# Keytoyze/Mug-Diffusion

Hardware: NVIDIA H100
Metric: denoising-steps/sec (higher is better)
Workload: dtype f32

## Files before the change

### include/mugd.h

```cpp
#ifndef MUGD_H
#define MUGD_H

#include <stdint.h>

#ifdef __cplusplus
extern "C" {
#endif

#define MUGD_ABI_VERSION 13

typedef struct mugd_handle mugd_handle;
typedef struct mugd_plan mugd_plan;

enum mugd_status {
    MUGD_OK = 0,
    MUGD_ERR_INVALID = 1,
    MUGD_ERR_CUDA = 2,
    MUGD_ERR_NO_DEVICE = 3,
    MUGD_ERR_OOM = 4
};

enum mugd_op_kind {
    MUGD_OP_GEMM = 1,
    MUGD_OP_GROUPNORM = 2,
    MUGD_OP_LAYERNORM = 3,
    MUGD_OP_ATTENTION = 4,
    MUGD_OP_S4CONV = 5,
    MUGD_OP_DDIM_UPDATE = 6,
    MUGD_OP_TRANSPOSE = 7,
    MUGD_OP_COPY2D = 8,
    MUGD_OP_STEP_ADVANCE = 9,
    MUGD_OP_NOTES = 10,
    MUGD_OP_EMBED = 11,
    MUGD_OP_TF32_SPLIT = 12,
    MUGD_OP_POSTERIOR = 13
};

enum mugd_conv_mode {
    MUGD_CONV_NONE = 0,
    MUGD_CONV_SAME = 1,
    MUGD_CONV_DOWN = 2,
    MUGD_CONV_UP = 3,
    MUGD_CONV_TAPS = 4
};
enum mugd_act { MUGD_ACT_NONE = 0, MUGD_ACT_SILU = 1, MUGD_ACT_GELU = 2 };
enum mugd_gate { MUGD_GATE_NONE = 0, MUGD_GATE_GEGLU = 1 ,
                 MUGD_GATE_GLU = 2  };
enum mugd_gemm_impl { MUGD_GEMM_AUTO = 0, MUGD_GEMM_SIMT = 1 ,
                      MUGD_GEMM_TC = 2  };

typedef struct mugd_gemm {
    const float* A;  int64_t lda;
    const float* W;
    const float* W_hi;
    const float* W_lo;
    const float* bias;
    const float* rowvec;
    int64_t rowvec_b_stride;
    int64_t rowvec_step_stride;
    const int32_t* step;
    const float* residual; int64_t ldr;
    float* C;        int64_t ldc;
    int32_t M, N, K;
    int32_t taps, conv_mode, Lin, Lout;
    int32_t act, gate, impl;
    int32_t split_k;
    int32_t n_counters;
    int32_t tap_shift;
    int32_t tap_dilation;
    void* workspace; int64_t workspace_bytes;
    int32_t* counters;
    const float* A2; int64_t lda2;
    int32_t K2; int32_t reserved_;
    double* row_moments;
    const double* ln_stats; const float* ln_colsum; float ln_eps; int32_t reserved2_;
} mugd_gemm;

typedef struct mugd_groupnorm {
    const float* x; int64_t ldx; float* y; int64_t ldy;
    const float* gamma; const float* beta;
    int32_t B, L, C, G; float eps; int32_t silu;
} mugd_groupnorm;

typedef struct mugd_layernorm {
    const float* x; int64_t ldx; float* y; int64_t ldy;
    const float* gamma; const float* beta;
    int32_t rows, C; float eps;
} mugd_layernorm;

typedef struct mugd_attention {
    const float* q; int64_t ldq;
    const float* k; int64_t ldk;
    const float* v; int64_t ldv;
    float* o; int64_t ldo;
    const float* relpos;
    const float* cgain;
    int32_t B, H, D, Lq, Lk, pos_max; float scale;
} mugd_attention;

typedef struct mugd_s4conv {
    const float* u; int64_t ldu;
    const float* Kt;
    const float* D;
    float* y; int64_t ldy;
    int32_t B, L, H;
} mugd_s4conv;

typedef struct mugd_ddim_update {
    float* x;
    float* x_dup;
    const float* eps;
    const float* noise;
    float* pred_x0;
    const float* coef;
    const int32_t* step;
    int32_t S; int32_t n;
    int32_t cfg; float scale; float temperature;
} mugd_ddim_update;

typedef struct mugd_transpose {
    const float* in; float* out;
    int64_t ldi, ldo; int32_t B, C, L, to_nlc;
} mugd_transpose;

typedef struct mugd_copy2d {
    const float* src; int64_t lds; float* dst; int64_t ldd; int32_t rows, cols;
} mugd_copy2d;

typedef struct mugd_step_advance { int32_t* step; } mugd_step_advance;

typedef struct mugd_notes {
    const float* logits; int64_t ld;
    int32_t* count; int32_t* start_ms; int32_t* end_ms;
    double frame_ms;
    int32_t B, T, K;
} mugd_notes;

typedef struct mugd_embed {
    const float* table;
    const int32_t* ids;
    float* out;
    int32_t B, F, H, n_embed;
} mugd_embed;

typedef struct mugd_tf32_split { float* w_hi; float* lo; int64_t n; } mugd_tf32_split;

typedef struct mugd_posterior {
    const float* params;
    const float* noise;
    float *mean, *logvar, *std, *z;
    float scale;
    int32_t B, Z, L;
} mugd_posterior;

typedef struct mugd_op {
    int32_t kind;
    int32_t tag;
    union {
        mugd_gemm gemm; mugd_groupnorm gn; mugd_layernorm ln; mugd_attention attn; mugd_s4conv s4;
        mugd_ddim_update ddim; mugd_transpose tr; mugd_copy2d cp; mugd_step_advance adv; mugd_notes notes;
        mugd_embed embed; mugd_tf32_split split; mugd_posterior post;
    } u;
} mugd_op;

int  mugd_abi_version(void);
const char* mugd_last_error(void);
int  mugd_create(int device, mugd_handle** out);
void mugd_destroy(mugd_handle* h);
int  mugd_device_info(mugd_handle* h, int32_t* sm_count, int32_t* cc_major, int32_t* cc_minor);
int  mugd_set_gemm_impl(mugd_handle* h, int impl);
int  mugd_set_pdl(int enabled);

int  mugd_op_run(mugd_handle* h, const mugd_op* op, void* stream);

int  mugd_plan_create(mugd_handle* h, const mugd_op* ops, int32_t n_ops, mugd_plan** out);
int  mugd_plan_run(mugd_plan* p, void* stream);
int  mugd_plan_capture(mugd_plan* p, void* stream);
int  mugd_plan_replay(mugd_plan* p, int32_t times, void* stream);
int  mugd_plan_launch_count(mugd_plan* p);
void mugd_plan_destroy(mugd_plan* p);

int  mugd_sample(mugd_plan* eval_plan, const mugd_op* tail, int32_t n_tail, int32_t n_steps, void* stream);

typedef struct mugd_stage {
    float* x; float* x_dup;
    const float* x0;
    const float* mask;
    const float* q_noise;
    const float* q_coef;
    const float* noise;
    float* noise_rows;
    int32_t B, C, L, reserved_;
} mugd_stage;
int  mugd_sample_staged(mugd_plan* eval_plan, const mugd_stage* stage, const mugd_op* tail, int32_t n_tail, int32_t n_steps,
                        void* stream);

typedef struct mugd_plms {
    mugd_ddim_update update;
    const float* eps;
    float* e_prime;
    float* hist;
    float* x_stash;
    int32_t cfg; float scale;
} mugd_plms;
int  mugd_sample_plms(mugd_plan* eval_plan, const mugd_plms* p, int32_t first_step, int32_t n_steps, void* stream);
int  mugd_plms_combine(const mugd_plms* p, int32_t step, int32_t heun, void* stream);

#define MUGD_MAX_STEPS 1000
typedef struct mugd_ddpm {
    float* x; float* x_dup;
    const float* eps;
    float* pred_x0;
    const float* noise;
    const float* coef;
    int32_t* step;
    int32_t T, B, C, L;
    int32_t cfg; float scale;
    int32_t clip;
    int32_t reserved_;
} mugd_ddpm;
int  mugd_sample_ddpm(mugd_plan* eval_plan, const mugd_ddpm* d, int32_t first_step, int32_t n_steps, void* stream);
int  mugd_ddpm_update(const mugd_ddpm* d, void* stream);

typedef struct mugd_dpm {
    float* x; float* x_dup;
    const float* eps;
    float* pred_x0;
    float* ring;
    const float* coef;
    int32_t* step;
    int32_t n, S;
    int32_t cfg; float scale;
} mugd_dpm;
int  mugd_sample_dpm(mugd_plan* eval_plan, const mugd_dpm* d, int32_t first_step, int32_t n_steps, void* stream);
int  mugd_dpm_update(const mugd_dpm* d, void* stream);

typedef struct mugd_dpm_ex {
    mugd_dpm dpm;
    const mugd_stage* stage;
    const int32_t* start;
    const float* order_coef;
    int32_t B, reserved_;
} mugd_dpm_ex;
int  mugd_sample_dpm_ex(mugd_plan* eval_plan, const mugd_dpm_ex* e, int32_t first_step, int32_t n_steps, void* stream);
int  mugd_dpm_ex_update(const mugd_dpm_ex* e, void* stream);

typedef struct mugd_dpm_stop {
    mugd_dpm dpm;
    const int32_t* stop;
    int32_t B, reserved_;
} mugd_dpm_stop;
int  mugd_sample_dpm_stop(mugd_plan* eval_plan, const mugd_dpm_stop* e, int32_t first_step, int32_t n_steps, void* stream);
int  mugd_dpm_stop_update(const mugd_dpm_stop* e, void* stream);

typedef struct mugd_unipc {
    mugd_dpm dpm;
    float* xc;
    const float* corr;
} mugd_unipc;
int  mugd_sample_unipc(mugd_plan* eval_plan, const mugd_unipc* u, int32_t first_step, int32_t n_steps, void* stream);
int  mugd_unipc_update(const mugd_unipc* u, void* stream);

typedef struct mugd_unipc_ex {
    mugd_unipc unipc;
    const mugd_stage* stage;
    const int32_t* start;
    const float* order_coef;
    const float* order_corr;
    int32_t B, reserved_;
} mugd_unipc_ex;
int  mugd_sample_unipc_ex(mugd_plan* eval_plan, const mugd_unipc_ex* e, int32_t first_step, int32_t n_steps, void* stream);
int  mugd_unipc_ex_update(const mugd_unipc_ex* e, void* stream);

typedef struct mugd_unipc_stop {
    mugd_unipc unipc;
    const int32_t* stop;
    int32_t B, reserved_;
} mugd_unipc_stop;
int  mugd_sample_unipc_stop(mugd_plan* eval_plan, const mugd_unipc_stop* e, int32_t first_step, int32_t n_steps, void* stream);
int  mugd_unipc_stop_update(const mugd_unipc_stop* e, void* stream);

typedef struct mugd_q_encode {
    const float* x0; const float* noise;
    const int64_t* t;
    const float* sqrt_a; const float* sqrt_1ma;
    float* out;
    int32_t B, C, L, n;
} mugd_q_encode;
int  mugd_stochastic_encode(const mugd_q_encode* d, void* stream);

typedef struct mugd_join {
    float* x; float* x_dup;
    const float* x_latent;
    const int32_t* join;
    int32_t B, C, L, reserved_;
} mugd_join;
int  mugd_sample_join(mugd_plan* eval_plan, const mugd_join* join, const mugd_op* tail, int32_t n_tail, int32_t first_step,
                      int32_t n_steps, void* stream);

typedef struct mugd_region { const char* name; void* base; int64_t bytes; } mugd_region;
int  mugd_plan_save(mugd_plan* p, const mugd_region* regions, int32_t n_regions, const char* path);
int  mugd_plan_load(mugd_handle* h, const char* path, const mugd_region* regions, int32_t n_regions, mugd_plan** out);
int  mugd_plan_ops(mugd_plan* p, const mugd_op** ops, int32_t* n_ops);
int  mugd_plan_regions(const char* path, mugd_region* out, char (*names)[48], int32_t max_regions, int32_t* n_regions);

int  mugd_s4_kernel_gen(mugd_handle* h,
                        const float* log_dt,
                        const float* Bri,
                        const float* Cri,
                        const float* Pri,
                        const float* inv_w_real,
                        const float* w_imag,
                        const float* omega_ri,
                        int32_t H, int32_t N, int32_t L_internal, int32_t L_out,
                        float* Kt,
                        void* workspace, int64_t workspace_bytes,
                        void* stream);

int  mugd_melspec(mugd_handle* h,
                  const float* y, int64_t n, int64_t ldy, int32_t B,
                  const double* window, const double* twiddle, int32_t n_fft,
                  const int32_t* band_start, const int32_t* band_len, const float* weights, int32_t n_mels,
                  int32_t hop,
                  float* out, int64_t ldo, int32_t T_out,
                  void* stream);

int  mugd_grid_scan(mugd_handle* h, const float* times, const int32_t* chart_start, int32_t n_charts,
                    const double* cands, int32_t n_cands,
                    const int32_t* k0, const int32_t* head_len, const double* best_off, const double* best_score,
                    const float* first, const double* head_bpm, const double* head_off,
                    void* workspace, int32_t* out_i, double* out_d, void* stream);

int  mugd_chart_snap(mugd_handle* h, const int32_t* times, const int32_t* chart_start, int32_t n_charts,
                     const double* bpm, const double* offset, const int32_t* offset_is_f32, int64_t* out, void* stream);

int  mugd_remove_mini_jacks(mugd_handle* h, const int32_t* chart_start, int32_t n_charts, double jack_interval,
                            const double* start, const double* end, const uint8_t* is_long, int32_t* x, uint8_t* state,
                            void* workspace, void* stream);

int  mugd_gemm_tc_query(mugd_handle* h, const mugd_gemm* g, int32_t sm_count, int32_t* supported, int32_t* splits,
                        int64_t* workspace_bytes, int32_t* n_tiles);
int  mugd_gemm_tc_variant(const mugd_gemm* g, int32_t sm_count, int32_t* tile_n, int32_t* ctas_per_sm, int32_t* grid_ctas);

int  mugd_set_tc_single_pass_tf32(mugd_handle* h, int enabled);

int  mugd_set_attention_impl(mugd_handle* h, int impl);

int  mugd_set_s4conv_impl(mugd_handle* h, int impl);

int  mugd_debug_set_tc_cost(float kstep128_us, float kstep256_us, float split_us, float two_cta_fixed_us);

int  mugd_debug_set_tc_tile_n(int bn);

int  mugd_debug_set_attention_dump(float* buf);

int  mugd_debug_set_tc_timing(long long* device_buf);

int  mugd_fill_i32(int32_t* dst, int32_t value, void* stream);
int  mugd_abi_sizes(int32_t* out, int32_t n);

#ifdef __cplusplus
}
#endif
#endif
```

### mug_diffusion_b200/csrc/gemm_tc.cu

```cuda
#include "gemm_tc.cuh"

namespace mugd {

template <int BN, int EPI>
__global__ void __launch_bounds__(TC_THREADS, 1)
gemm_tc_kernel(const __grid_constant__ CUtensorMap tmA, const __grid_constant__ CUtensorMap tmA1,
               const __grid_constant__ CUtensorMap tmA2, const __grid_constant__ CUtensorMap tmB, const __grid_constant__ CUtensorMap tmWhi,
               const __grid_constant__ CUtensorMap tmWlo, const __grid_constant__ TcParams p) {
    extern __shared__ uint8_t smem_raw[];
    const uint32_t base = (smem_u32(smem_raw) + 1023u) & ~1023u;
    const TcBars<BN> B(base);
    TC_STAMP(p, 0, blockIdx.x == 0 && blockIdx.y == 0 && blockIdx.z == 0);
    if (threadIdx.x < 32) {
        B.init_parallel((int)threadIdx.x);
    } else if (threadIdx.x < 38) {
        const CUtensorMap* m = threadIdx.x == 32 ? &tmA : threadIdx.x == 33 ? &tmA1 : threadIdx.x == 34 ? &tmA2
                             : threadIdx.x == 35 ? &tmB : threadIdx.x == 36 ? &tmWhi : &tmWlo;
        asm volatile("prefetch.tensormap [%0];" ::"l"(reinterpret_cast<uint64_t>(m)) : "memory");
    }
    __syncthreads();
    TC_STAMP(p, 1, blockIdx.x == 0 && blockIdx.y == 0 && blockIdx.z == 0);
    gemm_tc_tile<BN, EPI>(&tmA, &tmA1, &tmA2, &tmB, &tmWhi, &tmWlo, p, blockIdx.x, blockIdx.y, blockIdx.z, base);
}

template <int BN, int EPI>
__global__ void __launch_bounds__(TC_THREADS)
gemm_tc_reduce_kernel(const __grid_constant__ TcParams p) {
    tc_reduce<BN, EPI>(p, blockIdx.x);
}

#ifdef MUGD_TC_TIMELINE
static long long* g_tc_dbg = nullptr;
#endif
static float g_tc_kstep128 = 0.55f;
static float g_tc_split = 3.0f;
static int g_tc_force_bn = 0;

static bool tc_shape_ok(const mugd_gemm& g) {
    if (!(g.conv_mode == MUGD_CONV_NONE || g.conv_mode == MUGD_CONV_SAME || g.conv_mode == MUGD_CONV_DOWN ||
          g.conv_mode == MUGD_CONV_TAPS)) return false;
    if (g.conv_mode == MUGD_CONV_DOWN && g.Lout < 2) return false;
    if (g.K2 % TC_BK != 0 || (g.K2 > 0 && g.conv_mode == MUGD_CONV_DOWN)) return false;
    return g.K % TC_BK == 0 && g.N >= 16 && g.N % 4 == 0;
}

bool gemm_tc_supported(const mugd_gemm& g) {
    if (!tc_shape_ok(g)) return false;
    if (!g.W_hi || !g.W_lo) return false;
    if (g.lda % 4 != 0 || !aligned16(g.A) || !aligned16(g.W_hi) || !aligned16(g.W_lo)) return false;
    if (g.K2 > 0 && (!g.A2 || g.lda2 % 4 != 0 || !aligned16(g.A2))) return false;
    return true;
}

static int tc_validate_fusions(const mugd_gemm& g) {
    if (g.row_moments)
        MUGD_REQUIRE(g.act == MUGD_ACT_NONE && g.gate == MUGD_GATE_NONE && !g.ln_stats && (reinterpret_cast<uintptr_t>(g.row_moments) & 15u) == 0,
                     "gemm: row_moments needs act == gate == NONE, no folded LayerNorm and a 16-byte aligned buffer");
    if (g.ln_stats) {
        MUGD_REQUIRE(g.ln_colsum && aligned16(g.ln_colsum) && (reinterpret_cast<uintptr_t>(g.ln_stats) & 15u) == 0 && g.taps == 1 && g.K2 == 0 &&
                         g.act == MUGD_ACT_NONE && (g.gate == MUGD_GATE_NONE || g.gate == MUGD_GATE_GEGLU) && !g.rowvec,
                     "gemm: folded LayerNorm needs a single-source Linear with act NONE and gate NONE/GEGLU");
    }
    return MUGD_OK;
}

TcGeometry tc_geometry(const mugd_gemm& g, int sm_count, int forced_split) {
    TcGeometry t = {};
    TcParams::Hot& h = t.hot;
    t.BN = (g.N >= 128) ? 128 : 64;
    if (g.conv_mode == MUGD_CONV_NONE) { h.Lrows = g.M; h.Bs = 1; }
    else { h.Lrows = g.Lout; h.Bs = g.M / g.Lout; }
    if (h.Lrows >= TC_BM) {
        h.box_l = TC_BM; h.box_b = 1;
        h.tiles_per_sample = (h.Lrows + TC_BM - 1) / TC_BM;
        t.gy = h.tiles_per_sample * h.Bs;
    } else {
        h.box_l = h.Lrows;
        h.box_b = TC_BM / h.Lrows;
        if (h.box_b > h.Bs) h.box_b = h.Bs;
        h.tiles_per_sample = 1;
        t.gy = (h.Bs + h.box_b - 1) / h.box_b;
    }
    h.kblocks = g.K / TC_BK;
    h.it_main = g.taps * h.kblocks;
    h.total_it = h.it_main + g.K2 / TC_BK;
    int splits = 1;
    float best = 1e30f;
    static const int cands[2] = {64, 128};
    for (int cand = 0; cand < 2; ++cand) {
        const int bn = cands[cand];
        if (bn > 64 && g.N < bn) continue;
        if (bn == 64 && g.N >= 128 && g_tc_force_bn != 64) continue;
        if (g_tc_force_bn && bn != g_tc_force_bn && !(g_tc_force_bn > g.N && bn == 64)) continue;
        const int gx = (g.N + bn - 1) / bn;
        const int tiles = gx * t.gy;
        const float kstep = bn == 128 ? g_tc_kstep128 : 0.4f;
        const int sp_max = forced_split > 0 ? forced_split : (tiles < sm_count ? 16 : 1);
        for (int sp = forced_split > 0 ? forced_split : 1; sp <= sp_max && sp <= h.total_it; ++sp) {
            const int per = (h.total_it + sp - 1) / sp;
            if (forced_split <= 0 && sp > 1 && per < 2) break;
            if (forced_split <= 0 && sp > 1 && tiles * sp > 2 * sm_count) break;
            const int waves = (tiles * sp + sm_count - 1) / sm_count;
            const float est = waves * (1.0f + kstep * per) + (sp > 1 ? g_tc_split : 0.0f);
            if (est < best - 0.25f) { best = est; splits = sp; t.BN = bn; }
        }
    }
    h.gx = (g.N + t.BN - 1) / t.BN;
    if (splits > h.total_it) splits = h.total_it;
    if (splits < 1) splits = 1;
    h.splits = splits;
    h.it_base = h.total_it / splits;
    h.it_rem = h.total_it % splits;
    h.conv_mode = g.conv_mode;
    h.tap_shift = g.tap_shift;
    h.tap_dilation = g.tap_dilation;
    t.ws_floats = splits > 1 ? (int64_t)h.gx * t.gy * splits * TC_BM * t.BN : 0;
    return t;
}

int tc_plan(const DeviceInfo& dev, const mugd_gemm& g, const mugd_gemm* next, TcPlanned* out) {
    MUGD_REQUIRE(gemm_tc_supported(g), "gemm_tc: unsupported shape/operands");
    int rc = tc_validate_fusions(g);
    if (rc != MUGD_OK) return rc;
    const TcGeometry t = tc_geometry(g, dev.sm_count, g.split_k);
    const TcParams::Hot& h = t.hot;
    if (h.splits > 1) {
        MUGD_REQUIRE(g.workspace, "gemm_tc: split-K needs a workspace");
        MUGD_REQUIRE(g.workspace_bytes >= t.ws_floats * 4, "gemm_tc: workspace too small (%lld < %lld)", (long long)g.workspace_bytes,
                     (long long)t.ws_floats * 4);
    }
    const cuuint32_t a_box[3] = {(cuuint32_t)TC_BK, (cuuint32_t)h.box_l, (cuuint32_t)h.box_b};
    for (int tap = 0; tap < 3; ++tap) {
        if (tap > 0 && g.conv_mode != MUGD_CONV_DOWN) { out->maps[tap] = out->maps[0]; continue; }
        const bool down = g.conv_mode == MUGD_CONV_DOWN;
        const cuuint64_t rows = down ? (cuuint64_t)(h.Lrows - (tap == 2 ? 1 : 0)) : (cuuint64_t)h.Lrows;
        const cuuint64_t sample_rows = down ? (cuuint64_t)g.Lin : (cuuint64_t)h.Lrows;
        const cuuint64_t dims[3] = {(cuuint64_t)g.K, rows, (cuuint64_t)h.Bs};
        const cuuint64_t strides[2] = {(cuuint64_t)g.lda * 4 * (down ? 2 : 1), sample_rows * (cuuint64_t)g.lda * 4};
        rc = encode_f32_tma(&out->maps[tap], g.A + (down ? (int64_t)tap * g.lda : 0), 3, dims, strides, a_box, CU_TENSOR_MAP_L2_PROMOTION_L2_128B,
                            "gemm_tc A");
        if (rc != MUGD_OK) return rc;
    }
    if (g.K2 > 0) {
        const cuuint64_t dims[3] = {(cuuint64_t)g.K2, (cuuint64_t)h.Lrows, (cuuint64_t)h.Bs};
        const cuuint64_t strides[2] = {(cuuint64_t)g.lda2 * 4, (cuuint64_t)h.Lrows * (cuuint64_t)g.lda2 * 4};
        rc = encode_f32_tma(&out->maps[3], g.A2, 3, dims, strides, a_box, CU_TENSOR_MAP_L2_PROMOTION_L2_128B, "gemm_tc A2");
        if (rc != MUGD_OK) return rc;
    } else {
        out->maps[3] = out->maps[0];
    }
    const cuuint64_t ktot = (cuuint64_t)g.taps * g.K + g.K2;
    const cuuint64_t w_dims[2] = {ktot, (cuuint64_t)g.N};
    const cuuint64_t w_strides[1] = {ktot * 4};
    const cuuint32_t w_box[2] = {(cuuint32_t)TC_BK, (cuuint32_t)t.BN};
    for (int w = 0; w < 2; ++w) {
        rc = encode_f32_tma(&out->maps[4 + w], w == 0 ? g.W_hi : g.W_lo, 2, w_dims, w_strides, w_box, CU_TENSOR_MAP_L2_PROMOTION_L2_256B,
                            "gemm_tc W");
        if (rc != MUGD_OK) return rc;
    }
    TcParams& p = out->p;
    memset(&p, 0, sizeof(p));
    p.hot = h;
    p.hot.single_pass = dev.tc_single_pass ? 1 : 0;
    p.g = g;
    p.ws = (float*)g.workspace;
    p.gy = t.gy;
    p.ln_invK = 1.0 / (double)g.K;
    if (next) {
        p.pf_hi = next->W_hi;
        p.pf_lo = p.hot.single_pass ? nullptr : next->W_lo;
        p.pf_bytes = (int64_t)next->N * ((int64_t)next->taps * next->K + next->K2) * 4;
    }
#ifdef MUGD_TC_TIMELINE
    p.dbg = g_tc_dbg;
#endif
    out->BN = t.BN;
    return MUGD_OK;
}

template <int BN, int EPI>
static int tc_launch(const TcPlanned& pl, cudaStream_t st) {
    const TcParams& p = pl.p;
    const TcParams::Hot& h = p.hot;
    if (h.splits > 1) {
        MUGD_CHECK_CUDA(launch_k(gemm_tc_kernel<BN, TC_E_NONE>, dim3(h.gx, p.gy, h.splits), dim3(TC_THREADS), TcSmem<BN>::TOTAL, st, pl.maps[0],
                                 pl.maps[1], pl.maps[2], pl.maps[3], pl.maps[4], pl.maps[5], p));
        MUGD_CHECK_CUDA(launch_k(gemm_tc_reduce_kernel<BN, EPI>, dim3((unsigned)(h.gx * p.gy * (TC_BM / TC_RED_ROWS<BN>))), dim3(TC_THREADS), 0,
                                 st, p));
        return MUGD_OK;
    }
    MUGD_CHECK_CUDA(launch_k(gemm_tc_kernel<BN, EPI>, dim3(h.gx, p.gy, 1), dim3(TC_THREADS), TcSmem<BN>::TOTAL, st, pl.maps[0], pl.maps[1],
                             pl.maps[2], pl.maps[3], pl.maps[4], pl.maps[5], p));
    return MUGD_OK;
}

template <int BN, int... EPI>
static cudaError_t allow_smem_bn(int bytes, std::integer_sequence<int, EPI...>) {
    return allow_dynamic_smem(bytes, gemm_tc_kernel<BN, EPI>...);
}
cudaError_t gemm_tc_allow_smem(int bytes) {
    const cudaError_t e = allow_smem_bn<64>(bytes, std::make_integer_sequence<int, TC_E_COUNT>{});
    return e != cudaSuccess ? e : allow_smem_bn<128>(bytes, std::make_integer_sequence<int, TC_E_COUNT>{});
}

template <int BN>
static int tc_launch_bn(const TcPlanned& pl, cudaStream_t st) {
    switch (tc_epi_of(pl.p.g)) {
        case TC_E_GEGLU: return tc_launch<BN, TC_E_GEGLU>(pl, st);
        case TC_E_GLU: return tc_launch<BN, TC_E_GLU>(pl, st);
        case TC_E_SILU: return tc_launch<BN, TC_E_SILU>(pl, st);
        case TC_E_GELU: return tc_launch<BN, TC_E_GELU>(pl, st);
        case TC_E_SINK: return tc_launch<BN, TC_E_SINK>(pl, st);
        case TC_E_LN: return tc_launch<BN, TC_E_LN>(pl, st);
        case TC_E_LN_GEGLU: return tc_launch<BN, TC_E_LN_GEGLU>(pl, st);
        default: return tc_launch<BN, TC_E_NONE>(pl, st);
    }
}

int launch_gemm_tc(const DeviceInfo& dev, const mugd_gemm& g, const mugd_gemm* next, cudaStream_t st, int* launches) {
    TcPlanned pl;
    int rc = tc_plan(dev, g, next, &pl);
    if (rc != MUGD_OK) return rc;
    if (pl.BN == 128) rc = tc_launch_bn<128>(pl, st);
    else rc = tc_launch_bn<64>(pl, st);
    if (rc != MUGD_OK) return rc;
    if (launches) *launches += pl.p.hot.splits > 1 ? 2 : 1;
    return MUGD_OK;
}

}

extern "C" int mugd_debug_set_tc_cost(float kstep128_us, float kstep256_us, float split_us, float two_cta_fixed_us) {
    (void)kstep256_us;
    (void)two_cta_fixed_us;
    if (kstep128_us > 0.f) mugd::g_tc_kstep128 = kstep128_us;
    if (split_us > 0.f) mugd::g_tc_split = split_us;
    return MUGD_OK;
}

extern "C" int mugd_debug_set_tc_tile_n(int bn) {
    mugd::g_tc_force_bn = (bn == 64 || bn == 128) ? bn : 0;
    return MUGD_OK;
}

extern "C" int mugd_debug_set_tc_timing(long long* device_buf) {
#ifdef MUGD_TC_TIMELINE
    mugd::g_tc_dbg = device_buf;
    return MUGD_OK;
#else
    (void)device_buf;
    mugd::set_error("mugd_debug_set_tc_timing: this build has no timeline hooks (rebuild with -DMUGD_TC_TIMELINE, tools/build_variant.py)");
    return MUGD_ERR_INVALID;
#endif
}

extern "C" int mugd_gemm_tc_variant(const mugd_gemm* g, int32_t sm_count, int32_t* tile_n, int32_t* ctas_per_sm, int32_t* grid_ctas) {
    using namespace mugd;
    MUGD_REQUIRE(g, "gemm_tc_variant: null");
    if (!tc_shape_ok(*g)) {
        if (tile_n) *tile_n = 0;
        if (ctas_per_sm) *ctas_per_sm = 0;
        if (grid_ctas) *grid_ctas = 0;
        return MUGD_OK;
    }
    const int sms = sm_count > 0 ? sm_count : 132;
    const TcGeometry t = tc_geometry(*g, sms, g->split_k);
    if (tile_n) *tile_n = t.BN;
    if (ctas_per_sm) *ctas_per_sm = 1;
    if (grid_ctas) *grid_ctas = t.hot.gx * t.gy * t.hot.splits;
    return MUGD_OK;
}

extern "C" int mugd_gemm_tc_query(mugd_handle*, const mugd_gemm* g, int32_t sm_count, int32_t* supported, int32_t* splits,
                                  int64_t* workspace_bytes, int32_t* n_tiles) {
    using namespace mugd;
    MUGD_REQUIRE(g, "gemm_tc_query: null");
    const bool ok = tc_shape_ok(*g);
    if (supported) *supported = ok ? 1 : 0;
    if (!ok) {
        if (splits) *splits = 0;
        if (workspace_bytes) *workspace_bytes = 0;
        if (n_tiles) *n_tiles = 0;
        return MUGD_OK;
    }
    const TcGeometry t = tc_geometry(*g, sm_count > 0 ? sm_count : 132, g->split_k);
    if (splits) *splits = t.hot.splits;
    if (workspace_bytes) *workspace_bytes = t.ws_floats * 4;
    if (n_tiles) *n_tiles = t.hot.gx * t.gy;
    return MUGD_OK;
}
```

### mug_diffusion_b200/csrc/gemm_tc.cuh

```cuda
#pragma once
#include <cuda.h>
#include <stddef.h>

#include <type_traits>

#include "common.cuh"
#include "wgmma.cuh"

namespace mugd {

constexpr int TC_BM = 128;
constexpr int TC_BK = 32;
constexpr int TC_THREADS = 256;
constexpr uint32_t TC_A_BYTES = TC_BM * TC_BK * 4;

struct TcParams {
    struct Hot {
        int32_t Lrows, Bs;
        int32_t box_l, box_b;
        int32_t tiles_per_sample;
        int32_t it_base, it_rem;
        int32_t it_main;
        int32_t kblocks;
        int32_t total_it;
        int32_t splits;
        int32_t single_pass;
        int32_t conv_mode, tap_shift, tap_dilation;
        int32_t gx;
    } hot;
    mugd_gemm g;
    float* ws;
    int32_t gy;
    double ln_invK;
    const float* pf_hi;
    const float* pf_lo;
    int64_t pf_bytes;
#ifdef MUGD_TC_TIMELINE
    long long* dbg;
#endif
};
static_assert(sizeof(TcParams::Hot) == 64 && offsetof(TcParams, hot) == 0, "the hot fields are the first 64 bytes of the parameters");

#ifdef __CUDACC__
__device__ __forceinline__ long long gtimer() {
    long long t;
    asm volatile("mov.u64 %0, %%globaltimer;" : "=l"(t) :: "memory");
    return t;
}
#ifdef MUGD_TC_TIMELINE
#define TC_STAMP(p, k, cta0) do { if ((p).dbg && (cta0) && threadIdx.x == 0) (p).dbg[k] = gtimer(); } while (0)
#else
#define TC_STAMP(p, k, cta0) do { } while (0)
#endif
template <int BN>
struct TcSmem {
    static_assert(BN == 64 || BN == 128, "tile widths of the wgmma kernel");
    static constexpr uint32_t B_BYTES = BN * TC_BK * 4;
    static constexpr uint32_t STAGE_BYTES = TC_A_BYTES + 2 * B_BYTES;
    static constexpr int STAGES = BN == 128 ? 4 : 6;
    static constexpr uint32_t TILE_BYTES = STAGES * STAGE_BYTES;
    static constexpr uint32_t BAR_BYTES = 256;
    static constexpr uint32_t TOTAL = TILE_BYTES + 1024  + BAR_BYTES;
    static_assert(TOTAL <= 227u * 1024u, "shared memory budget");
    static_assert(128u * (BN + 4) * 4u + 1024u <= TILE_BYTES, "the staged accumulator tile + row statistics must fit the pipeline buffers");
};

template <int SEG>
__device__ __forceinline__ void tc_row_sink(double* buf, int m, float4 v) {
    float s = (v.x + v.y) + (v.z + v.w);
    float ss = (v.x * v.x + v.y * v.y) + (v.z * v.z + v.w * v.w);
#pragma unroll
    for (int o = SEG / 2; o > 0; o >>= 1) {
        s += __shfl_xor_sync(0xffffffffu, s, o);
        ss += __shfl_xor_sync(0xffffffffu, ss, o);
    }
    if ((threadIdx.x & (SEG - 1)) == 0 && m >= 0) {
        atomicAdd(buf + (int64_t)m * 2, (double)s);
        atomicAdd(buf + (int64_t)m * 2 + 1, (double)ss);
    }
}
__device__ __forceinline__ float2 tc_ln_from_moments(double s, double ss, double invK, float eps) {
    const double mean = s * invK;
    double var = ss * invK - mean * mean;
    const float v = fmaxf((float)var, 0.f) + eps;
    float r = rsqrtf(v);
    r = r * (1.5f - 0.5f * v * r * r);
    return make_float2((float)mean, r);
}

constexpr int TC_EPI_PLAIN = 0, TC_EPI_SINK = 1 , TC_EPI_LN = 2 ;

template <int ACT, int GATE, bool LNF>
__device__ __forceinline__ float4 tc_finish4(const mugd_gemm& g, float* dst, float4 acc, float4 bia, float4 rvv, float4 res, float4 cs, float2 ln,
                                             int m, int no) {
    float x[4];
    if constexpr (LNF) {
        x[0] = (acc.x - ln.x * cs.x) * ln.y + bia.x + rvv.x; x[1] = (acc.y - ln.x * cs.y) * ln.y + bia.y + rvv.y;
        x[2] = (acc.z - ln.x * cs.z) * ln.y + bia.z + rvv.z; x[3] = (acc.w - ln.x * cs.w) * ln.y + bia.w + rvv.w;
    } else {
        x[0] = acc.x + bia.x + rvv.x; x[1] = acc.y + bia.y + rvv.y; x[2] = acc.z + bia.z + rvv.z; x[3] = acc.w + bia.w + rvv.w;
    }
    if constexpr (ACT == MUGD_ACT_SILU) {
#pragma unroll
        for (int j = 0; j < 4; ++j) x[j] = silu_f(x[j]);
    } else if constexpr (ACT == MUGD_ACT_GELU) {
#pragma unroll
        for (int j = 0; j < 4; ++j) x[j] = gelu_f(x[j]);
    }
    if constexpr (GATE == MUGD_GATE_NONE) {
        const float4 o = make_float4(x[0] + res.x, x[1] + res.y, x[2] + res.z, x[3] + res.w);
        st_f4(dst, o);
        return o;
    } else {
        float o0, o1;
        if constexpr (GATE == MUGD_GATE_GEGLU) { o0 = x[0] * gelu_f(x[1]); o1 = x[2] * gelu_f(x[3]); }
        else { o0 = x[0] * sigmoid_f(x[1]); o1 = x[2] * sigmoid_f(x[3]); }
        if (g.residual) {
            const float2 rr = *reinterpret_cast<const float2*>(g.residual + (int64_t)m * g.ldr + no);
            o0 += rr.x; o1 += rr.y;
        }
        *reinterpret_cast<float2*>(dst) = make_float2(o0, o1);
        return make_float4(o0, o1, 0.f, 0.f);
    }
}

template <int BN, int ACT, int GATE, int MODE>
__device__ __forceinline__ void tc_store_tile(const mugd_gemm& g, uint32_t stage, int m_base, int n0, int rows_valid, const float* rowvec,
                                              uint32_t rowstat, float4 bia, float4 cs) {
    constexpr int SP = BN + 4;
    constexpr int C4 = BN / 4;
    constexpr int NU = TC_BM * C4 / TC_THREADS;
    constexpr int U = NU < 16 ? NU : 16;
    constexpr int SEG = C4 < 32 ? C4 : 32;
    static_assert(TC_THREADS % C4 == 0, "a thread keeps its column quad for the whole tile");
    const int c4 = (int)threadIdx.x % C4;
    const int nn = n0 + c4 * 4;
    const bool col_ok = nn < g.N;
    const bool has_res = GATE == MUGD_GATE_NONE && g.residual != nullptr;
    constexpr int RPP = TC_THREADS / C4;
    const int row0 = (int)threadIdx.x / C4;
    const int n_rows = min(rows_valid, g.M - m_base);
    const int no = (GATE == MUGD_GATE_NONE) ? nn : (nn >> 1);
    float* cp = g.C + (int64_t)(m_base + row0) * g.ldc + no;
    const float* rp = has_res ? g.residual + (int64_t)(m_base + row0) * g.ldr + nn : nullptr;
    const int64_t c_step = (int64_t)RPP * g.ldc, r_step = (int64_t)RPP * g.ldr;
    int smp = 0, smp_end = 0;
    if (rowvec) { smp = (m_base + row0) / g.Lout; smp_end = (smp + 1) * g.Lout; }
    auto pass = [&](auto full_tag) {
        constexpr bool FULL = decltype(full_tag)::value;
#pragma unroll 1
        for (int i0 = 0; i0 < NU; i0 += U) {
            float4 res[U], rvv[U];
#pragma unroll
            for (int u = 0; u < U; ++u) {
                const int row = row0 + (i0 + u) * RPP;
                res[u] = rvv[u] = make_float4(0.f, 0.f, 0.f, 0.f);
                if (FULL || (row < n_rows && col_ok)) {
                    if (has_res) res[u] = ld_f4(rp + (int64_t)(i0 + u) * r_step);
                    if (rowvec) {
                        const int m = m_base + row;
                        while (m >= smp_end) { ++smp; smp_end += g.Lout; }
                        rvv[u] = ld_f4(rowvec + (int64_t)smp * g.rowvec_b_stride + nn);
                    }
                }
            }
#pragma unroll
            for (int u = 0; u < U; ++u) {
                const int row = row0 + (i0 + u) * RPP;
                const int m = m_base + row;
                const bool ok = FULL || (row < n_rows && col_ok);
                const float4 acc = lds_f4(stage + (uint32_t)(row * SP + c4 * 4) * 4u);
                float2 ln = make_float2(0.f, 1.f);
                if constexpr (MODE == TC_EPI_LN) ln = lds_f2(rowstat + (uint32_t)row * 8u);
                float4 o = make_float4(0.f, 0.f, 0.f, 0.f);
                if (ok) o = tc_finish4<ACT, GATE, MODE == TC_EPI_LN>(g, cp + (int64_t)(i0 + u) * c_step, acc, bia, rvv[u], res[u], cs, ln, m, no);
                if constexpr (MODE == TC_EPI_SINK) tc_row_sink<SEG>(g.row_moments, ok ? m : -1, o);
            }
        }
    };
    if (n_rows >= TC_BM && n0 + BN <= g.N) pass(std::true_type{});
    else pass(std::false_type{});
}

enum TcEpi { TC_E_NONE = 0, TC_E_GEGLU, TC_E_GLU, TC_E_SILU, TC_E_GELU, TC_E_SINK, TC_E_LN, TC_E_LN_GEGLU, TC_E_COUNT };
template <int EPI> struct TcEpiTraits;
template <> struct TcEpiTraits<TC_E_NONE>     { static constexpr int ACT = MUGD_ACT_NONE, GATE = MUGD_GATE_NONE,  MODE = TC_EPI_PLAIN; };
template <> struct TcEpiTraits<TC_E_GEGLU>    { static constexpr int ACT = MUGD_ACT_NONE, GATE = MUGD_GATE_GEGLU, MODE = TC_EPI_PLAIN; };
template <> struct TcEpiTraits<TC_E_GLU>      { static constexpr int ACT = MUGD_ACT_NONE, GATE = MUGD_GATE_GLU,   MODE = TC_EPI_PLAIN; };
template <> struct TcEpiTraits<TC_E_SILU>     { static constexpr int ACT = MUGD_ACT_SILU, GATE = MUGD_GATE_NONE,  MODE = TC_EPI_PLAIN; };
template <> struct TcEpiTraits<TC_E_GELU>     { static constexpr int ACT = MUGD_ACT_GELU, GATE = MUGD_GATE_NONE,  MODE = TC_EPI_PLAIN; };
template <> struct TcEpiTraits<TC_E_SINK>     { static constexpr int ACT = MUGD_ACT_NONE, GATE = MUGD_GATE_NONE,  MODE = TC_EPI_SINK; };
template <> struct TcEpiTraits<TC_E_LN>       { static constexpr int ACT = MUGD_ACT_NONE, GATE = MUGD_GATE_NONE,  MODE = TC_EPI_LN; };
template <> struct TcEpiTraits<TC_E_LN_GEGLU> { static constexpr int ACT = MUGD_ACT_NONE, GATE = MUGD_GATE_GEGLU, MODE = TC_EPI_LN; };

inline int tc_epi_of(const mugd_gemm& g) {
    if (g.ln_stats) return g.gate == MUGD_GATE_GEGLU ? TC_E_LN_GEGLU : TC_E_LN;
    if (g.row_moments) return TC_E_SINK;
    if (g.gate == MUGD_GATE_GEGLU) return TC_E_GEGLU;
    if (g.gate == MUGD_GATE_GLU) return TC_E_GLU;
    if (g.act == MUGD_ACT_SILU) return TC_E_SILU;
    if (g.act == MUGD_ACT_GELU) return TC_E_GELU;
    return TC_E_NONE;
}

__device__ __forceinline__ void tc_tile_rows(const TcParams& p, int by, int& b_base, int& l_base, int& rows_valid) {
    const TcParams::Hot& h = p.hot;
    if (h.Lrows >= TC_BM) {
        b_base = by / h.tiles_per_sample;
        l_base = (by % h.tiles_per_sample) * TC_BM;
        rows_valid = min(TC_BM, h.Lrows - l_base);
    } else {
        b_base = by * h.box_b;
        l_base = 0;
        rows_valid = min(h.box_b, h.Bs - b_base) * h.Lrows;
    }
}

template <int BN>
struct TcBars {
    using S = TcSmem<BN>;
    static constexpr int COUNT = 2 * S::STAGES;
    static_assert(8 * COUNT <= (int)S::BAR_BYTES, "barrier block");
    uint32_t bars;
    __device__ __forceinline__ explicit TcBars(uint32_t base) : bars(base + S::TILE_BYTES) {}
    __device__ __forceinline__ uint32_t full(int s) const { return bars + 8u * s; }
    __device__ __forceinline__ uint32_t empty(int s) const { return bars + 8u * (S::STAGES + s); }
    __device__ __forceinline__ void init_parallel(int t) const {
        if (t >= COUNT) return;
        mbar_init(bars + 8u * t, t < S::STAGES ? 1u : (uint32_t)(TC_THREADS / 32));
        mbar_init_fence();
    }
};

struct TcAFrag {
    uint32_t hi[4][4], lo[4][4];
};
__device__ __forceinline__ void tc_load_split(uint32_t a_tile, int r0, int t, TcAFrag& f) {
#pragma unroll
    for (int kk = 0; kk < 4; ++kk) {
#pragma unroll
        for (int e = 0; e < 4; ++e) {
            const int r = r0 + (e & 1) * 8;
            const int chunk = 2 * kk + (e >> 1);
            const float x = lds_f1(a_tile + (uint32_t)r * 128u + (uint32_t)((chunk ^ (r & 7)) << 4) + (uint32_t)t * 4u);
            const float h = to_tf32(x);
            f.hi[kk][e] = __float_as_uint(h);
            f.lo[kk][e] = __float_as_uint(to_tf32(x - h));
        }
    }
}

template <int BN, int EPI>
__device__ __forceinline__ void gemm_tc_tile(const CUtensorMap* tmA, const CUtensorMap* tmA1, const CUtensorMap* tmA2, const CUtensorMap* tmB,
                                             const CUtensorMap* tmWhi, const CUtensorMap* tmWlo, const TcParams& p, int bx, int by, int bz,
                                             uint32_t base) {
    using S = TcSmem<BN>;
    constexpr int STAGES = S::STAGES;
    constexpr int NACC = BN / 2;
    const TcBars<BN> B(base);
    auto a_raw = [&](int s) { return base + s * S::STAGE_BYTES; };
    auto b_hi = [&](int s) { return base + s * S::STAGE_BYTES + TC_A_BYTES; };
    auto b_lo = [&](int s) { return b_hi(s) + S::B_BYTES; };

    const mugd_gemm& g = p.g;
    const TcParams::Hot& h = p.hot;
    const int warp = threadIdx.x >> 5, lane = threadIdx.x & 31;
    const int n0 = bx * BN;
    int b_base, l_base, rows_valid;
    tc_tile_rows(p, by, b_base, l_base, rows_valid);
    const int m_base = b_base * h.Lrows + l_base;
    const int it_begin = bz * h.it_base + min(bz, h.it_rem);
    const int nit = h.it_base + (bz < h.it_rem ? 1 : 0);
    const uint32_t a_tx = (uint32_t)(h.box_l * h.box_b) * TC_BK * 4;
    const uint32_t w_tx = (h.single_pass ? 1u : 2u) * S::B_BYTES;

    auto issue_w = [&](int i) {
        const int s = i % STAGES, it = it_begin + i;
        mbar_expect_tx(B.full(s), a_tx + w_tx);
        tma_load_2d(b_hi(s), tmWhi, B.full(s), it * TC_BK, n0);
        if (!h.single_pass) tma_load_2d(b_lo(s), tmWlo, B.full(s), it * TC_BK, n0);
    };
    auto issue_a = [&](int i) {
        const int s = i % STAGES, it = it_begin + i;
        if (it < h.it_main) {
            const int t = it / h.kblocks;
            const int kb = it - t * h.kblocks;
            const CUtensorMap* ma = tmA;
            int lshift = 0;
            if (h.conv_mode == MUGD_CONV_SAME) lshift = t - 1;
            else if (h.conv_mode == MUGD_CONV_TAPS) lshift = (t + h.tap_shift) * (h.tap_dilation > 1 ? h.tap_dilation : 1);
            else if (h.conv_mode == MUGD_CONV_DOWN) ma = (t == 0) ? tmA : (t == 1 ? tmA1 : tmA2);
            tma_load_3d(a_raw(s), ma, B.full(s), kb * TC_BK, l_base + lshift, b_base);
        } else {
            tma_load_3d(a_raw(s), tmB, B.full(s), (it - h.it_main) * TC_BK, l_base, b_base);
        }
    };
    if (warp == 0) {
        if (elect_one()) {
            const int pro = nit < STAGES ? nit : STAGES;
            for (int i = 0; i < pro; ++i) issue_w(i);
            pdl_wait();
            for (int i = 0; i < pro; ++i) issue_a(i);
            if (p.pf_bytes > 0) {
                const int64_t ncta = (int64_t)h.gx * p.gy * h.splits;
                const int64_t per = (p.pf_bytes / ncta + 15) & ~(int64_t)15;
                const int64_t off = (((int64_t)bz * p.gy + by) * h.gx + bx) * per;
                const int64_t n = min(per, p.pf_bytes - off);
                if (n > 0) {
                    prefetch_l2(reinterpret_cast<const char*>(p.pf_hi) + off, (uint32_t)n);
                    if (p.pf_lo) prefetch_l2(reinterpret_cast<const char*>(p.pf_lo) + off, (uint32_t)n);
                }
            }
        }
        __syncwarp();
    }

    int epi_step = 0;
    float4 epi_bias = make_float4(0.f, 0.f, 0.f, 0.f), epi_cs = epi_bias;
    double ln_s = 0.0, ln_ss = 0.0;
    {
        pdl_wait();
        if (h.splits == 1) {
            const int nn = n0 + ((int)threadIdx.x % (BN / 4)) * 4;
            if (g.step) epi_step = *g.step;
            if (g.bias && nn < g.N) epi_bias = ld_f4(g.bias + nn);
            if constexpr (TcEpiTraits<EPI>::MODE == TC_EPI_LN) {
                if (nn < g.N) epi_cs = ld_f4(g.ln_colsum + nn);
            }
        }
        if constexpr (TcEpiTraits<EPI>::MODE == TC_EPI_LN) {
            const int rr = (int)threadIdx.x;
            if (rr < TC_BM && rr < rows_valid && m_base + rr < g.M) {
                const double2 mo = *reinterpret_cast<const double2*>(g.ln_stats + (int64_t)m_base * 2 + rr * 2);
                ln_s = mo.x; ln_ss = mo.y;
            }
        }
    }

    const int wg = warp >> 2, g8 = lane >> 2, t4 = lane & 3;
    const int r0 = wg * 64 + (warp & 3) * 16 + g8;
    float acc[NACC];
#pragma unroll
    for (int j = 0; j < NACC; ++j) acc[j] = 0.f;
    TcAFrag f0, f1;
    if (nit > 0) {
        mbar_wait(B.full(0), 0u);
        tc_load_split(a_raw(0), r0, t4, f0);
    }
    auto main_loop = [&](auto single_tag) {
        constexpr bool SINGLE = decltype(single_tag)::value;
        auto kstep = [&](int i, const TcAFrag& cur, TcAFrag& nxt) {
            const int s = i % STAGES;
            const uint64_t dbh = wgmma_desc(b_hi(s)), dbl = wgmma_desc(b_lo(s));
            wgmma_fence();
#pragma unroll
            for (int kk = 0; kk < TC_BK / 8; ++kk) {
                const uint64_t ko = (uint64_t)(kk * 2);
                if constexpr (SINGLE) {
                    Wgmma<BN>::mma(acc, cur.hi[kk], dbh + ko);
                } else {
                    Wgmma<BN>::mma(acc, cur.lo[kk], dbh + ko);
                    Wgmma<BN>::mma(acc, cur.hi[kk], dbl + ko);
                    Wgmma<BN>::mma(acc, cur.hi[kk], dbh + ko);
                }
            }
            wgmma_commit();
            wgmma_wait<1>();
            if (i > 0) {
                const int j = i - 1, sj = j % STAGES;
                __syncwarp();
                if (lane == 0) mbar_arrive(B.empty(sj));
                if (warp == 0 && j + STAGES < nit) {
                    mbar_wait(B.empty(sj), (uint32_t)(j / STAGES) & 1u);
                    if (elect_one()) { issue_w(j + STAGES); issue_a(j + STAGES); }
                    __syncwarp();
                }
            }
            if (i + 1 < nit) {
                mbar_wait(B.full((i + 1) % STAGES), (uint32_t)((i + 1) / STAGES) & 1u);
                tc_load_split(a_raw((i + 1) % STAGES), r0, t4, nxt);
            }
        };
        for (int i = 0; i < nit; i += 2) {
            kstep(i, f0, f1);
            if (i + 1 < nit) kstep(i + 1, f1, f0);
        }
    };
    if (h.single_pass) main_loop(std::true_type{});
    else main_loop(std::false_type{});
    wgmma_wait<0>();
    TC_STAMP(p, 2, bx == 0 && by == 0 && bz == 0);
    float2 lnrow = make_float2(0.f, 1.f);
    if constexpr (TcEpiTraits<EPI>::MODE == TC_EPI_LN) lnrow = tc_ln_from_moments(ln_s, ln_ss, p.ln_invK, g.ln_eps);
    __syncthreads();
    constexpr int SP = BN + 4;
#pragma unroll
    for (int j = 0; j < BN / 8; ++j) {
        const int c = j * 8 + 2 * t4;
        sts_f2(base + (uint32_t)(r0 * SP + c) * 4u, acc[4 * j], acc[4 * j + 1]);
        sts_f2(base + (uint32_t)((r0 + 8) * SP + c) * 4u, acc[4 * j + 2], acc[4 * j + 3]);
    }
    if constexpr (TcEpiTraits<EPI>::MODE == TC_EPI_LN) {
        if (threadIdx.x < TC_BM) sts_f2(base + S::TILE_BYTES - 1024u + (uint32_t)threadIdx.x * 8u, lnrow.x, lnrow.y);
    }
    __syncthreads();
    TC_STAMP(p, 3, bx == 0 && by == 0 && bz == 0);
    {
        const float* rowvec = g.rowvec ? g.rowvec + (int64_t)epi_step * g.rowvec_step_stride : nullptr;
        if (h.splits > 1) {
            const int tile_lin = by * h.gx + bx;
            float* wsp = p.ws + ((int64_t)tile_lin * h.splits + bz) * (TC_BM * BN);
            constexpr int C4 = BN / 4;
            constexpr int U = 8;
#pragma unroll 1
            for (int i0 = 0; i0 < TC_BM * C4; i0 += TC_THREADS * U) {
                float4 a4[U];
#pragma unroll
                for (int u = 0; u < U; ++u) {
                    const int idx = i0 + u * TC_THREADS + (int)threadIdx.x;
                    const int row = idx / C4, c4 = idx - row * C4;
                    a4[u] = lds_f4(base + (uint32_t)(row * SP + c4 * 4) * 4u);
                }
#pragma unroll
                for (int u = 0; u < U; ++u) st_f4(wsp + (i0 + u * TC_THREADS + (int)threadIdx.x) * 4, a4[u]);
            }
        } else {
            using E = TcEpiTraits<EPI>;
            tc_store_tile<BN, E::ACT, E::GATE, E::MODE>(g, base, m_base, n0, rows_valid, rowvec, base + S::TILE_BYTES - 1024u, epi_bias, epi_cs);
        }
    }
    TC_STAMP(p, 4, bx == 0 && by == 0 && bz == 0);
}

template <int BN> constexpr int TC_RED_ROWS = TC_THREADS / (BN / 4);

template <int BN, int EPI>
__device__ __forceinline__ void tc_reduce(const TcParams& p, int blk) {
    constexpr int ACT = TcEpiTraits<EPI>::ACT, GATE = TcEpiTraits<EPI>::GATE, MODE = TcEpiTraits<EPI>::MODE;
    constexpr int C4 = BN / 4;
    constexpr int BPT = TC_BM / TC_RED_ROWS<BN>;
    constexpr int SEG = C4 < 32 ? C4 : 32;
    constexpr int ZU = 8;
    const mugd_gemm& g = p.g;
    const TcParams::Hot& h = p.hot;
    const int tile_lin = blk / BPT;
    const int bx = tile_lin % h.gx, by = tile_lin / h.gx;
    int b_base, l_base, rows_valid;
    tc_tile_rows(p, by, b_base, l_base, rows_valid);
    const int m_base = b_base * h.Lrows + l_base;
    const int c4 = (int)threadIdx.x % C4;
    const int r = (blk % BPT) * TC_RED_ROWS<BN> + (int)threadIdx.x / C4;
    const int n = bx * BN + c4 * 4;
    const int m = m_base + r;
    const bool ok = r < rows_valid && m < g.M && n < g.N;
    float4 bia = make_float4(0.f, 0.f, 0.f, 0.f), rvv = bia, res = bia, cs = bia;
    if (ok && g.bias) bia = ld_f4(g.bias + n);
    if constexpr (MODE == TC_EPI_LN) {
        if (ok) cs = ld_f4(g.ln_colsum + n);
    }
    pdl_wait();
    int step = 0;
    if (g.step) step = *g.step;
    if (GATE == MUGD_GATE_NONE && g.residual && ok) res = ld_f4(g.residual + (int64_t)m * g.ldr + n);
    double2 mo = make_double2(0.0, 1.0);
    if constexpr (MODE == TC_EPI_LN) {
        if (ok) mo = *reinterpret_cast<const double2*>(g.ln_stats + (int64_t)m * 2);
    }
    const float* src = p.ws + ((long long)tile_lin * h.splits) * (TC_BM * BN) + (long long)r * BN + c4 * 4;
    float4 acc = make_float4(0.f, 0.f, 0.f, 0.f);
    for (int z0 = 0; z0 < h.splits; z0 += ZU) {
        float4 t4[ZU];
#pragma unroll
        for (int u = 0; u < ZU; ++u) {
            t4[u] = make_float4(0.f, 0.f, 0.f, 0.f);
            if (ok && z0 + u < h.splits) t4[u] = __ldcg(reinterpret_cast<const float4*>(src + (long long)(z0 + u) * (TC_BM * BN)));
        }
        if (z0 == 0 && g.rowvec && ok)
            rvv = ld_f4(g.rowvec + (int64_t)step * g.rowvec_step_stride + (int64_t)(m / g.Lout) * g.rowvec_b_stride + n);
#pragma unroll
        for (int u = 0; u < ZU; ++u) { acc.x += t4[u].x; acc.y += t4[u].y; acc.z += t4[u].z; acc.w += t4[u].w; }
    }
    float4 o = make_float4(0.f, 0.f, 0.f, 0.f);
    if (ok) {
        float2 ln = make_float2(0.f, 1.f);
        if constexpr (MODE == TC_EPI_LN) ln = tc_ln_from_moments(mo.x, mo.y, p.ln_invK, g.ln_eps);
        const int no = (GATE == MUGD_GATE_NONE) ? n : (n >> 1);
        o = tc_finish4<ACT, GATE, MODE == TC_EPI_LN>(g, g.C + (int64_t)m * g.ldc + no, acc, bia, rvv, res, cs, ln, m, no);
    }
    if constexpr (MODE == TC_EPI_SINK) tc_row_sink<SEG>(g.row_moments, ok ? m : -1, o);
}

#endif

struct TcGeometry {
    TcParams::Hot hot;
    int BN, gy;
    int64_t ws_floats;
};
struct alignas(64) TcPlanned {
    CUtensorMap maps[6];
    TcParams p;
    int BN;
};
TcGeometry tc_geometry(const mugd_gemm& g, int sm_count, int forced_split);
int tc_plan(const DeviceInfo& dev, const mugd_gemm& g, const mugd_gemm* next, TcPlanned* out);

}
```

### mug_diffusion_b200/lib.py

```python
from __future__ import annotations

import ctypes as C
import os
from typing import Optional

HERE = os.path.dirname(os.path.abspath(__file__))
LIB_PATH = os.environ.get("MUGD_LIB") or os.path.join(HERE, "libmugd.so")

(OP_GEMM, OP_GROUPNORM, OP_LAYERNORM, OP_ATTENTION, OP_S4CONV, OP_DDIM_UPDATE, OP_TRANSPOSE, OP_COPY2D, OP_STEP_ADVANCE, OP_NOTES, OP_EMBED,
 OP_TF32_SPLIT, OP_POSTERIOR) = range(1, 14)
CONV_NONE, CONV_SAME, CONV_DOWN, CONV_UP, CONV_TAPS = range(5)
ACT_NONE, ACT_SILU, ACT_GELU = range(3)
GATE_NONE, GATE_GEGLU, GATE_GLU = range(3)
GEMM_AUTO, GEMM_SIMT, GEMM_TC = range(3)
ABI_VERSION = 13

_f = C.c_void_p


class Gemm(C.Structure):
    _fields_ = [("A", _f), ("lda", C.c_int64), ("W", _f), ("W_hi", _f), ("W_lo", _f), ("bias", _f), ("rowvec", _f),
                ("rowvec_b_stride", C.c_int64), ("rowvec_step_stride", C.c_int64), ("step", _f),
                ("residual", _f), ("ldr", C.c_int64), ("C", _f), ("ldc", C.c_int64),
                ("M", C.c_int32), ("N", C.c_int32), ("K", C.c_int32),
                ("taps", C.c_int32), ("conv_mode", C.c_int32), ("Lin", C.c_int32), ("Lout", C.c_int32),
                ("act", C.c_int32), ("gate", C.c_int32), ("impl", C.c_int32),
                ("split_k", C.c_int32), ("n_counters", C.c_int32), ("tap_shift", C.c_int32), ("tap_dilation", C.c_int32),
                ("workspace", _f), ("workspace_bytes", C.c_int64), ("counters", _f),
                ("A2", _f), ("lda2", C.c_int64), ("K2", C.c_int32), ("reserved_", C.c_int32),
                ("row_moments", _f),
                ("ln_stats", _f), ("ln_colsum", _f), ("ln_eps", C.c_float), ("reserved2_", C.c_int32)]


class GroupNorm(C.Structure):
    _fields_ = [("x", _f), ("ldx", C.c_int64), ("y", _f), ("ldy", C.c_int64), ("gamma", _f), ("beta", _f),
                ("B", C.c_int32), ("L", C.c_int32), ("C", C.c_int32), ("G", C.c_int32),
                ("eps", C.c_float), ("silu", C.c_int32)]


class LayerNorm(C.Structure):
    _fields_ = [("x", _f), ("ldx", C.c_int64), ("y", _f), ("ldy", C.c_int64), ("gamma", _f), ("beta", _f),
                ("rows", C.c_int32), ("C", C.c_int32), ("eps", C.c_float)]


class Attention(C.Structure):
    _fields_ = [("q", _f), ("ldq", C.c_int64), ("k", _f), ("ldk", C.c_int64), ("v", _f), ("ldv", C.c_int64),
                ("o", _f), ("ldo", C.c_int64), ("relpos", _f), ("cgain", _f),
                ("B", C.c_int32), ("H", C.c_int32), ("D", C.c_int32), ("Lq", C.c_int32), ("Lk", C.c_int32),
                ("pos_max", C.c_int32), ("scale", C.c_float)]


class S4Conv(C.Structure):
    _fields_ = [("u", _f), ("ldu", C.c_int64), ("Kt", _f), ("D", _f), ("y", _f), ("ldy", C.c_int64),
                ("B", C.c_int32), ("L", C.c_int32), ("H", C.c_int32)]


class DdimUpdate(C.Structure):
    _fields_ = [("x", _f), ("x_dup", _f), ("eps", _f), ("noise", _f), ("pred_x0", _f), ("coef", _f), ("step", _f),
                ("S", C.c_int32), ("n", C.c_int32), ("cfg", C.c_int32), ("scale", C.c_float),
                ("temperature", C.c_float)]


class Transpose(C.Structure):
    _fields_ = [("inp", _f), ("out", _f), ("ldi", C.c_int64), ("ldo", C.c_int64),
                ("B", C.c_int32), ("C", C.c_int32), ("L", C.c_int32), ("to_nlc", C.c_int32)]


class Copy2D(C.Structure):
    _fields_ = [("src", _f), ("lds", C.c_int64), ("dst", _f), ("ldd", C.c_int64),
                ("rows", C.c_int32), ("cols", C.c_int32)]


class StepAdvance(C.Structure):
    _fields_ = [("step", _f)]


class Notes(C.Structure):
    _fields_ = [("logits", _f), ("ld", C.c_int64), ("count", _f), ("start_ms", _f), ("end_ms", _f), ("frame_ms", C.c_double),
                ("B", C.c_int32), ("T", C.c_int32), ("K", C.c_int32)]


class Embed(C.Structure):
    _fields_ = [("table", _f), ("ids", _f), ("out", _f), ("B", C.c_int32), ("F", C.c_int32), ("H", C.c_int32), ("n_embed", C.c_int32)]


class Tf32Split(C.Structure):
    _fields_ = [("w_hi", _f), ("lo", _f), ("n", C.c_int64)]


class Posterior(C.Structure):
    _fields_ = [("params", _f), ("noise", _f), ("mean", _f), ("logvar", _f), ("std", _f), ("z", _f), ("scale", C.c_float),
                ("B", C.c_int32), ("Z", C.c_int32), ("L", C.c_int32)]


class Stage(C.Structure):
    _fields_ = [("x", _f), ("x_dup", _f), ("x0", _f), ("mask", _f), ("q_noise", _f), ("q_coef", _f), ("noise", _f), ("noise_rows", _f),
                ("B", C.c_int32), ("C", C.c_int32), ("L", C.c_int32), ("reserved_", C.c_int32)]


class Plms(C.Structure):
    _fields_ = [("update", DdimUpdate), ("eps", _f), ("e_prime", _f), ("hist", _f), ("x_stash", _f), ("cfg", C.c_int32),
                ("scale", C.c_float)]


class Ddpm(C.Structure):
    _fields_ = [("x", _f), ("x_dup", _f), ("eps", _f), ("pred_x0", _f), ("noise", _f), ("coef", _f), ("step", _f),
                ("T", C.c_int32), ("B", C.c_int32), ("C", C.c_int32), ("L", C.c_int32), ("cfg", C.c_int32), ("scale", C.c_float),
                ("clip", C.c_int32), ("reserved_", C.c_int32)]


class Dpm(C.Structure):
    _fields_ = [("x", _f), ("x_dup", _f), ("eps", _f), ("pred_x0", _f), ("ring", _f), ("coef", _f), ("step", _f),
                ("n", C.c_int32), ("S", C.c_int32), ("cfg", C.c_int32), ("scale", C.c_float)]


class DpmEx(C.Structure):
    _fields_ = [("dpm", Dpm), ("stage", _f), ("start", _f), ("order_coef", _f), ("B", C.c_int32), ("reserved_", C.c_int32)]


class DpmStop(C.Structure):
    _fields_ = [("dpm", Dpm), ("stop", _f), ("B", C.c_int32), ("reserved_", C.c_int32)]


class Unipc(C.Structure):
    _fields_ = [("dpm", Dpm), ("xc", _f), ("corr", _f)]


class UnipcEx(C.Structure):
    _fields_ = [("unipc", Unipc), ("stage", _f), ("start", _f), ("order_coef", _f), ("order_corr", _f), ("B", C.c_int32),
                ("reserved_", C.c_int32)]


class UnipcStop(C.Structure):
    _fields_ = [("unipc", Unipc), ("stop", _f), ("B", C.c_int32), ("reserved_", C.c_int32)]


class QEncode(C.Structure):
    _fields_ = [("x0", _f), ("noise", _f), ("t", _f), ("sqrt_a", _f), ("sqrt_1ma", _f), ("out", _f),
                ("B", C.c_int32), ("C", C.c_int32), ("L", C.c_int32), ("n", C.c_int32)]


class Join(C.Structure):
    _fields_ = [("x", _f), ("x_dup", _f), ("x_latent", _f), ("join", _f),
                ("B", C.c_int32), ("C", C.c_int32), ("L", C.c_int32), ("reserved_", C.c_int32)]


class _OpU(C.Union):
    _fields_ = [("gemm", Gemm), ("gn", GroupNorm), ("ln", LayerNorm), ("attn", Attention), ("s4", S4Conv),
                ("ddim", DdimUpdate), ("tr", Transpose), ("cp", Copy2D), ("adv", StepAdvance), ("notes", Notes), ("embed", Embed),
                ("split", Tf32Split), ("post", Posterior)]


class Op(C.Structure):
    _fields_ = [("kind", C.c_int32), ("tag", C.c_int32), ("u", _OpU)]


_KIND_FIELD = {OP_GEMM: "gemm", OP_GROUPNORM: "gn", OP_LAYERNORM: "ln", OP_ATTENTION: "attn", OP_S4CONV: "s4",
               OP_DDIM_UPDATE: "ddim", OP_TRANSPOSE: "tr", OP_COPY2D: "cp", OP_STEP_ADVANCE: "adv", OP_NOTES: "notes", OP_EMBED: "embed", OP_TF32_SPLIT: "split",
               OP_POSTERIOR: "post"}


def make_op(kind: int, desc, tag: int = 0) -> Op:
    op = Op()
    op.kind = kind
    op.tag = tag
    setattr(op.u, _KIND_FIELD[kind], desc)
    return op


class Region(C.Structure):
    _fields_ = [("name", C.c_char_p), ("base", _f), ("bytes", C.c_int64)]


class MugdError(RuntimeError):
    pass


_lib: Optional[C.CDLL] = None


def load() -> C.CDLL:
    global _lib
    if _lib is not None:
        return _lib
    if not os.path.exists(LIB_PATH):
        raise MugdError(f"{LIB_PATH} not found: build it with `python -m mug_diffusion_b200.build` "
                        "(there is no CPU/PyTorch fallback for the sampler path)")
    lib = C.CDLL(LIB_PATH)
    lib.mugd_last_error.restype = C.c_char_p
    lib.mugd_abi_version.restype = C.c_int
    lib.mugd_create.argtypes = [C.c_int, C.POINTER(C.c_void_p)]
    lib.mugd_destroy.argtypes = [C.c_void_p]
    lib.mugd_destroy.restype = None
    lib.mugd_device_info.argtypes = [C.c_void_p, C.POINTER(C.c_int32), C.POINTER(C.c_int32), C.POINTER(C.c_int32)]
    lib.mugd_set_gemm_impl.argtypes = [C.c_void_p, C.c_int]
    lib.mugd_op_run.argtypes = [C.c_void_p, C.POINTER(Op), C.c_void_p]
    lib.mugd_plan_create.argtypes = [C.c_void_p, C.POINTER(Op), C.c_int32, C.POINTER(C.c_void_p)]
    lib.mugd_plan_run.argtypes = [C.c_void_p, C.c_void_p]
    lib.mugd_plan_capture.argtypes = [C.c_void_p, C.c_void_p]
    lib.mugd_plan_replay.argtypes = [C.c_void_p, C.c_int32, C.c_void_p]
    lib.mugd_plan_launch_count.argtypes = [C.c_void_p]
    lib.mugd_plan_destroy.argtypes = [C.c_void_p]
    lib.mugd_plan_destroy.restype = None
    lib.mugd_s4_kernel_gen.argtypes = [C.c_void_p] + [C.c_void_p] * 7 + [C.c_int32] * 4 + [C.c_void_p, C.c_void_p, C.c_int64, C.c_void_p]
    lib.mugd_melspec.argtypes = [C.c_void_p, C.c_void_p, C.c_int64, C.c_int64, C.c_int32, C.c_void_p, C.c_void_p, C.c_int32,
                                 C.POINTER(C.c_int32), C.POINTER(C.c_int32), C.c_void_p, C.c_int32, C.c_int32,
                                 C.c_void_p, C.c_int64, C.c_int32, C.c_void_p]
    lib.mugd_grid_scan.argtypes = [C.c_void_p, C.c_void_p, C.c_void_p, C.c_int32, C.c_void_p, C.c_int32] + [C.c_void_p] * 11
    lib.mugd_chart_snap.argtypes = [C.c_void_p, C.c_void_p, C.c_void_p, C.c_int32] + [C.c_void_p] * 5
    lib.mugd_remove_mini_jacks.argtypes = [C.c_void_p, C.c_void_p, C.c_int32, C.c_double] + [C.c_void_p] * 7
    lib.mugd_gemm_tc_variant.argtypes =[C.POINTER(Gemm), C.c_int32, C.POINTER(C.c_int32), C.POINTER(C.c_int32), C.POINTER(C.c_int32)]
    lib.mugd_gemm_tc_query.argtypes = [C.c_void_p, C.POINTER(Gemm), C.c_int32, C.POINTER(C.c_int32), C.POINTER(C.c_int32),
                                       C.POINTER(C.c_int64), C.POINTER(C.c_int32)]
    lib.mugd_set_pdl.argtypes = [C.c_int]
    lib.mugd_debug_set_tc_timing.argtypes = [C.c_void_p]
    lib.mugd_fill_i32.argtypes = [C.c_void_p, C.c_int32, C.c_void_p]
    lib.mugd_abi_sizes.argtypes = [C.POINTER(C.c_int32), C.c_int32]
    if lib.mugd_abi_version() != ABI_VERSION:
        raise MugdError(f"libmugd ABI {lib.mugd_abi_version()} != binding {ABI_VERSION}: rebuild the library")
    sizes = (C.c_int32 * 13)()
    lib.mugd_abi_sizes(sizes, 13)
    mine = [C.sizeof(t) for t in (Op, Gemm, GroupNorm, LayerNorm, Attention, S4Conv, DdimUpdate, Transpose, Copy2D, Notes, Embed, Tf32Split,
                                  Posterior)]
    if list(sizes) != mine:
        raise MugdError(f"struct layout mismatch: C {list(sizes)} vs ctypes {mine}")
    lib.mugd_sample.argtypes = [C.c_void_p, C.POINTER(Op), C.c_int32, C.c_int32, C.c_void_p]
    lib.mugd_sample_staged.argtypes = [C.c_void_p, C.POINTER(Stage), C.POINTER(Op), C.c_int32, C.c_int32, C.c_void_p]
    lib.mugd_sample_plms.argtypes = [C.c_void_p, C.POINTER(Plms), C.c_int32, C.c_int32, C.c_void_p]
    lib.mugd_plms_combine.argtypes = [C.POINTER(Plms), C.c_int32, C.c_int32, C.c_void_p]
    lib.mugd_sample_ddpm.argtypes = [C.c_void_p, C.POINTER(Ddpm), C.c_int32, C.c_int32, C.c_void_p]
    lib.mugd_ddpm_update.argtypes = [C.POINTER(Ddpm), C.c_void_p]
    lib.mugd_sample_dpm.argtypes = [C.c_void_p, C.POINTER(Dpm), C.c_int32, C.c_int32, C.c_void_p]
    lib.mugd_dpm_update.argtypes = [C.POINTER(Dpm), C.c_void_p]
    lib.mugd_sample_dpm_ex.argtypes = [C.c_void_p, C.POINTER(DpmEx), C.c_int32, C.c_int32, C.c_void_p]
    lib.mugd_dpm_ex_update.argtypes = [C.POINTER(DpmEx), C.c_void_p]
    lib.mugd_sample_dpm_stop.argtypes = [C.c_void_p, C.POINTER(DpmStop), C.c_int32, C.c_int32, C.c_void_p]
    lib.mugd_dpm_stop_update.argtypes = [C.POINTER(DpmStop), C.c_void_p]
    lib.mugd_sample_unipc.argtypes = [C.c_void_p, C.POINTER(Unipc), C.c_int32, C.c_int32, C.c_void_p]
    lib.mugd_unipc_update.argtypes = [C.POINTER(Unipc), C.c_void_p]
    lib.mugd_sample_unipc_ex.argtypes = [C.c_void_p, C.POINTER(UnipcEx), C.c_int32, C.c_int32, C.c_void_p]
    lib.mugd_unipc_ex_update.argtypes = [C.POINTER(UnipcEx), C.c_void_p]
    lib.mugd_sample_unipc_stop.argtypes = [C.c_void_p, C.POINTER(UnipcStop), C.c_int32, C.c_int32, C.c_void_p]
    lib.mugd_unipc_stop_update.argtypes = [C.POINTER(UnipcStop), C.c_void_p]
    lib.mugd_stochastic_encode.argtypes = [C.POINTER(QEncode), C.c_void_p]
    lib.mugd_sample_join.argtypes = [C.c_void_p, C.POINTER(Join), C.POINTER(Op), C.c_int32, C.c_int32, C.c_int32, C.c_void_p]
    lib.mugd_plan_save.argtypes = [C.c_void_p, C.POINTER(Region), C.c_int32, C.c_char_p]
    lib.mugd_plan_load.argtypes = [C.c_void_p, C.c_char_p, C.POINTER(Region), C.c_int32, C.POINTER(C.c_void_p)]
    lib.mugd_set_tc_single_pass_tf32.argtypes = [C.c_void_p, C.c_int]
    lib.mugd_set_attention_impl.argtypes = [C.c_void_p, C.c_int]
    lib.mugd_set_s4conv_impl.argtypes = [C.c_void_p, C.c_int]
    lib.mugd_debug_set_tc_tile_n.argtypes = [C.c_int]
    lib.mugd_debug_set_tc_cost.argtypes = [C.c_float, C.c_float, C.c_float, C.c_float]
    if os.environ.get("MUGD_TC_COST"):
        lib.mugd_debug_set_tc_cost(*([float(v) for v in os.environ["MUGD_TC_COST"].split(",")] + [0.0] * 4)[:4])
    if os.environ.get("MUGD_TC_TILE"):
        lib.mugd_debug_set_tc_tile_n(int(os.environ["MUGD_TC_TILE"]))
    if os.environ.get("MUGD_TC_BN"):
        lib.mugd_debug_set_tc_tile_n(int(os.environ["MUGD_TC_BN"]))
    if os.environ.get("MUGD_PDL") in ("0", "1"):
        lib.mugd_set_pdl(int(os.environ["MUGD_PDL"]))
    _lib = lib
    return lib


def check(rc: int, what: str = ""):
    if rc != 0:
        msg = load().mugd_last_error().decode(errors="replace")
        if rc == 4:
            import torch
            raise torch.cuda.OutOfMemoryError(f"{what}: {msg}")
        raise MugdError(f"{what} failed (status {rc}): {msg}")


EXPORTED_SYMBOLS = [
    "mugd_abi_version", "mugd_last_error", "mugd_create", "mugd_destroy", "mugd_device_info", "mugd_set_gemm_impl",
    "mugd_op_run", "mugd_plan_create", "mugd_plan_run", "mugd_plan_capture", "mugd_plan_replay",
    "mugd_plan_launch_count", "mugd_plan_destroy", "mugd_s4_kernel_gen", "mugd_fill_i32", "mugd_abi_sizes", "mugd_gemm_tc_query",
    "mugd_set_pdl", "mugd_set_tc_single_pass_tf32", "mugd_set_attention_impl", "mugd_set_s4conv_impl", "mugd_debug_set_tc_tile_n", "mugd_debug_set_tc_cost", "mugd_gemm_tc_variant",
    "mugd_debug_set_attention_dump", "mugd_debug_set_tc_timing", "mugd_sample", "mugd_plan_save", "mugd_plan_load", "mugd_plan_regions", "mugd_plan_ops",
    "mugd_melspec", "mugd_grid_scan", "mugd_chart_snap", "mugd_remove_mini_jacks",
    "mugd_sample_staged", "mugd_sample_plms", "mugd_plms_combine",
    "mugd_sample_ddpm", "mugd_ddpm_update", "mugd_stochastic_encode", "mugd_sample_join",
    "mugd_sample_dpm", "mugd_dpm_update", "mugd_sample_dpm_ex", "mugd_dpm_ex_update",
    "mugd_sample_dpm_stop", "mugd_dpm_stop_update",
    "mugd_sample_unipc", "mugd_unipc_update", "mugd_sample_unipc_ex", "mugd_unipc_ex_update",
    "mugd_sample_unipc_stop", "mugd_unipc_stop_update",
]
```

Measured before the change: 244.8.

## Add 256-row wgmma tile variant chosen by an L2-aware cost model

Adds a BM=256, BN=128 tile shape to the TF32 wgmma GEMM. Each warp holds two 64-row accumulator blocks so every weight tile loaded from shared memory is reused across twice as many rows. The geometry planner now compares 128- and 256-row candidates with a cost model that weighs tensor throughput against L2 bandwidth. The larger tile cuts the pipeline to 3 stages, raises register pressure, and is not split along K unless forced, which can reduce parallelism on small GEMMs.

```diff
diff --git a/include/mugd.h b/include/mugd.h
--- a/include/mugd.h
+++ b/include/mugd.h
@@ -352,6 +352,8 @@
 
 int  mugd_debug_set_tc_tile_n(int bn);
 
+int  mugd_debug_set_tc_tile_m(int bm);
+
 int  mugd_debug_set_attention_dump(float* buf);
 
 int  mugd_debug_set_tc_timing(long long* device_buf);
diff --git a/mug_diffusion_b200/csrc/gemm_tc.cu b/mug_diffusion_b200/csrc/gemm_tc.cu
--- a/mug_diffusion_b200/csrc/gemm_tc.cu
+++ b/mug_diffusion_b200/csrc/gemm_tc.cu
@@ -2,14 +2,14 @@
 
 namespace mugd {
 
-template <int BN, int EPI>
+template <int BM, int BN, int EPI>
 __global__ void __launch_bounds__(TC_THREADS, 1)
 gemm_tc_kernel(const __grid_constant__ CUtensorMap tmA, const __grid_constant__ CUtensorMap tmA1,
                const __grid_constant__ CUtensorMap tmA2, const __grid_constant__ CUtensorMap tmB, const __grid_constant__ CUtensorMap tmWhi,
                const __grid_constant__ CUtensorMap tmWlo, const __grid_constant__ TcParams p) {
     extern __shared__ uint8_t smem_raw[];
     const uint32_t base = (smem_u32(smem_raw) + 1023u) & ~1023u;
-    const TcBars<BN> B(base);
+    const TcBars<BM, BN> B(base);
     TC_STAMP(p, 0, blockIdx.x == 0 && blockIdx.y == 0 && blockIdx.z == 0);
     if (threadIdx.x < 32) {
         B.init_parallel((int)threadIdx.x);
@@ -20,13 +20,13 @@
     }
     __syncthreads();
     TC_STAMP(p, 1, blockIdx.x == 0 && blockIdx.y == 0 && blockIdx.z == 0);
-    gemm_tc_tile<BN, EPI>(&tmA, &tmA1, &tmA2, &tmB, &tmWhi, &tmWlo, p, blockIdx.x, blockIdx.y, blockIdx.z, base);
-}
-
-template <int BN, int EPI>
+    gemm_tc_tile<BM, BN, EPI>(&tmA, &tmA1, &tmA2, &tmB, &tmWhi, &tmWlo, p, blockIdx.x, blockIdx.y, blockIdx.z, base);
+}
+
+template <int BM, int BN, int EPI>
 __global__ void __launch_bounds__(TC_THREADS)
 gemm_tc_reduce_kernel(const __grid_constant__ TcParams p) {
-    tc_reduce<BN, EPI>(p, blockIdx.x);
+    tc_reduce<BM, BN, EPI>(p, blockIdx.x);
 }
 
 #ifdef MUGD_TC_TIMELINE
@@ -34,7 +34,10 @@
 #endif
 static float g_tc_kstep128 = 0.55f;
 static float g_tc_split = 3.0f;
+static float g_tc_tensor128_us = 0.78f;
+static float g_tc_l2_gbps = 5600.f;
 static int g_tc_force_bn = 0;
+static int g_tc_force_bm = 0;
 
 static bool tc_shape_ok(const mugd_gemm& g) {
     if (!(g.conv_mode == MUGD_CONV_NONE || g.conv_mode == MUGD_CONV_SAME || g.conv_mode == MUGD_CONV_DOWN ||
@@ -64,47 +67,64 @@
     return MUGD_OK;
 }
 
+static float tc_kstep_us(float tensor, float kbytes, int streams) {
+    const float l2 = kbytes * 1024.f * (float)streams / (g_tc_l2_gbps * 1e3f);
+    return tensor > l2 ? tensor : l2;
+}
+
 TcGeometry tc_geometry(const mugd_gemm& g, int sm_count, int forced_split) {
     TcGeometry t = {};
     TcParams::Hot& h = t.hot;
+    t.BM = 128;
     t.BN = (g.N >= 128) ? 128 : 64;
     if (g.conv_mode == MUGD_CONV_NONE) { h.Lrows = g.M; h.Bs = 1; }
     else { h.Lrows = g.Lout; h.Bs = g.M / g.Lout; }
-    if (h.Lrows >= TC_BM) {
-        h.box_l = TC_BM; h.box_b = 1;
-        h.tiles_per_sample = (h.Lrows + TC_BM - 1) / TC_BM;
-        t.gy = h.tiles_per_sample * h.Bs;
-    } else {
-        h.box_l = h.Lrows;
-        h.box_b = TC_BM / h.Lrows;
-        if (h.box_b > h.Bs) h.box_b = h.Bs;
-        h.tiles_per_sample = 1;
-        t.gy = (h.Bs + h.box_b - 1) / h.box_b;
-    }
+    auto row_tiles = [&](int bm) {
+        if (h.Lrows >= bm) return h.Bs * ((h.Lrows + bm - 1) / bm);
+        const int bb = bm / h.Lrows < h.Bs ? bm / h.Lrows : h.Bs;
+        return (h.Bs + bb - 1) / bb;
+    };
     h.kblocks = g.K / TC_BK;
     h.it_main = g.taps * h.kblocks;
     h.total_it = h.it_main + g.K2 / TC_BK;
     int splits = 1;
     float best = 1e30f;
-    static const int cands[2] = {64, 128};
-    for (int cand = 0; cand < 2; ++cand) {
-        const int bn = cands[cand];
+    static const int cand_bm[3] = {128, 128, 256}, cand_bn[3] = {64, 128, 128};
+    for (int cand = 0; cand < 3; ++cand) {
+        const int bm = cand_bm[cand], bn = cand_bn[cand];
         if (bn > 64 && g.N < bn) continue;
         if (bn == 64 && g.N >= 128 && g_tc_force_bn != 64) continue;
         if (g_tc_force_bn && bn != g_tc_force_bn && !(g_tc_force_bn > g.N && bn == 64)) continue;
+        if (g_tc_force_bm && bm != g_tc_force_bm && bn == 128) continue;
+        const int gy = row_tiles(bm);
         const int gx = (g.N + bn - 1) / bn;
-        const int tiles = gx * t.gy;
-        const float kstep = bn == 128 ? g_tc_kstep128 : 0.4f;
+        const int tiles = gx * gy;
         const int sp_max = forced_split > 0 ? forced_split : (tiles < sm_count ? 16 : 1);
         for (int sp = forced_split > 0 ? forced_split : 1; sp <= sp_max && sp <= h.total_it; ++sp) {
+            if (bm == 256 && sp > 1 && g_tc_force_bm != 256) break;
             const int per = (h.total_it + sp - 1) / sp;
             if (forced_split <= 0 && sp > 1 && per < 2) break;
             if (forced_split <= 0 && sp > 1 && tiles * sp > 2 * sm_count) break;
             const int waves = (tiles * sp + sm_count - 1) / sm_count;
+            float kstep = bn == 128 ? g_tc_kstep128 : 0.4f;
+            if (bm == 256) {
+                const int streams = tiles * sp < sm_count ? tiles * sp : sm_count;
+                kstep *= tc_kstep_us(2.f * g_tc_tensor128_us, 64.f, streams) / tc_kstep_us(g_tc_tensor128_us, 48.f, streams);
+            }
             const float est = waves * (1.0f + kstep * per) + (sp > 1 ? g_tc_split : 0.0f);
-            if (est < best - 0.25f) { best = est; splits = sp; t.BN = bn; }
+            if (est < best - 0.25f) { best = est; splits = sp; t.BM = bm; t.BN = bn; t.gy = gy; }
         }
     }
+    if (h.Lrows >= t.BM) {
+        h.box_l = t.BM; h.box_b = 1;
+        h.tiles_per_sample = (h.Lrows + t.BM - 1) / t.BM;
+    } else {
+        h.box_l = h.Lrows;
+        h.box_b = t.BM / h.Lrows;
+        if (h.box_b > h.Bs) h.box_b = h.Bs;
+        h.tiles_per_sample = 1;
+    }
+    t.gy = row_tiles(t.BM);
     h.gx = (g.N + t.BN - 1) / t.BN;
     if (splits > h.total_it) splits = h.total_it;
     if (splits < 1) splits = 1;
@@ -114,7 +134,7 @@
     h.conv_mode = g.conv_mode;
     h.tap_shift = g.tap_shift;
     h.tap_dilation = g.tap_dilation;
-    t.ws_floats = splits > 1 ? (int64_t)h.gx * t.gy * splits * TC_BM * t.BN : 0;
+    t.ws_floats = splits > 1 ? (int64_t)h.gx * t.gy * splits * t.BM * t.BN : 0;
     return t;
 }
 
@@ -174,46 +194,49 @@
 #ifdef MUGD_TC_TIMELINE
     p.dbg = g_tc_dbg;
 #endif
+    out->BM = t.BM;
     out->BN = t.BN;
     return MUGD_OK;
 }
 
-template <int BN, int EPI>
+template <int BM, int BN, int EPI>
 static int tc_launch(const TcPlanned& pl, cudaStream_t st) {
     const TcParams& p = pl.p;
     const TcParams::Hot& h = p.hot;
     if (h.splits > 1) {
-        MUGD_CHECK_CUDA(launch_k(gemm_tc_kernel<BN, TC_E_NONE>, dim3(h.gx, p.gy, h.splits), dim3(TC_THREADS), TcSmem<BN>::TOTAL, st, pl.maps[0],
-                                 pl.maps[1], pl.maps[2], pl.maps[3], pl.maps[4], pl.maps[5], p));
-        MUGD_CHECK_CUDA(launch_k(gemm_tc_reduce_kernel<BN, EPI>, dim3((unsigned)(h.gx * p.gy * (TC_BM / TC_RED_ROWS<BN>))), dim3(TC_THREADS), 0,
+        MUGD_CHECK_CUDA(launch_k(gemm_tc_kernel<BM, BN, TC_E_NONE>, dim3(h.gx, p.gy, h.splits), dim3(TC_THREADS), TcSmem<BM, BN>::TOTAL, st,
+                                 pl.maps[0], pl.maps[1], pl.maps[2], pl.maps[3], pl.maps[4], pl.maps[5], p));
+        MUGD_CHECK_CUDA(launch_k(gemm_tc_reduce_kernel<BM, BN, EPI>, dim3((unsigned)(h.gx * p.gy * (BM / TC_RED_ROWS<BN>))), dim3(TC_THREADS), 0,
                                  st, p));
         return MUGD_OK;
     }
-    MUGD_CHECK_CUDA(launch_k(gemm_tc_kernel<BN, EPI>, dim3(h.gx, p.gy, 1), dim3(TC_THREADS), TcSmem<BN>::TOTAL, st, pl.maps[0], pl.maps[1],
+    MUGD_CHECK_CUDA(launch_k(gemm_tc_kernel<BM, BN, EPI>, dim3(h.gx, p.gy, 1), dim3(TC_THREADS), TcSmem<BM, BN>::TOTAL, st, pl.maps[0], pl.maps[1],
                              pl.maps[2], pl.maps[3], pl.maps[4], pl.maps[5], p));
     return MUGD_OK;
 }
 
-template <int BN, int... EPI>
-static cudaError_t allow_smem_bn(int bytes, std::integer_sequence<int, EPI...>) {
-    return allow_dynamic_smem(bytes, gemm_tc_kernel<BN, EPI>...);
+template <int BM, int BN, int... EPI>
+static cudaError_t allow_smem_shape(int bytes, std::integer_sequence<int, EPI...>) {
+    return allow_dynamic_smem(bytes, gemm_tc_kernel<BM, BN, EPI>...);
 }
 cudaError_t gemm_tc_allow_smem(int bytes) {
-    const cudaError_t e = allow_smem_bn<64>(bytes, std::make_integer_sequence<int, TC_E_COUNT>{});
-    return e != cudaSuccess ? e : allow_smem_bn<128>(bytes, std::make_integer_sequence<int, TC_E_COUNT>{});
-}
-
-template <int BN>
-static int tc_launch_bn(const TcPlanned& pl, cudaStream_t st) {
+    using Seq = std::make_integer_sequence<int, TC_E_COUNT>;
+    cudaError_t e = allow_smem_shape<128, 64>(bytes, Seq{});
+    if (e == cudaSuccess) e = allow_smem_shape<128, 128>(bytes, Seq{});
+    return e != cudaSuccess ? e : allow_smem_shape<256, 128>(bytes, Seq{});
+}
+
+template <int BM, int BN>
+static int tc_launch_shape(const TcPlanned& pl, cudaStream_t st) {
     switch (tc_epi_of(pl.p.g)) {
-        case TC_E_GEGLU: return tc_launch<BN, TC_E_GEGLU>(pl, st);
-        case TC_E_GLU: return tc_launch<BN, TC_E_GLU>(pl, st);
-        case TC_E_SILU: return tc_launch<BN, TC_E_SILU>(pl, st);
-        case TC_E_GELU: return tc_launch<BN, TC_E_GELU>(pl, st);
-        case TC_E_SINK: return tc_launch<BN, TC_E_SINK>(pl, st);
-        case TC_E_LN: return tc_launch<BN, TC_E_LN>(pl, st);
-        case TC_E_LN_GEGLU: return tc_launch<BN, TC_E_LN_GEGLU>(pl, st);
-        default: return tc_launch<BN, TC_E_NONE>(pl, st);
+        case TC_E_GEGLU: return tc_launch<BM, BN, TC_E_GEGLU>(pl, st);
+        case TC_E_GLU: return tc_launch<BM, BN, TC_E_GLU>(pl, st);
+        case TC_E_SILU: return tc_launch<BM, BN, TC_E_SILU>(pl, st);
+        case TC_E_GELU: return tc_launch<BM, BN, TC_E_GELU>(pl, st);
+        case TC_E_SINK: return tc_launch<BM, BN, TC_E_SINK>(pl, st);
+        case TC_E_LN: return tc_launch<BM, BN, TC_E_LN>(pl, st);
+        case TC_E_LN_GEGLU: return tc_launch<BM, BN, TC_E_LN_GEGLU>(pl, st);
+        default: return tc_launch<BM, BN, TC_E_NONE>(pl, st);
     }
 }
 
@@ -221,8 +244,9 @@
     TcPlanned pl;
     int rc = tc_plan(dev, g, next, &pl);
     if (rc != MUGD_OK) return rc;
-    if (pl.BN == 128) rc = tc_launch_bn<128>(pl, st);
-    else rc = tc_launch_bn<64>(pl, st);
+    if (pl.BM == 256) rc = tc_launch_shape<256, 128>(pl, st);
+    else if (pl.BN == 128) rc = tc_launch_shape<128, 128>(pl, st);
+    else rc = tc_launch_shape<128, 64>(pl, st);
     if (rc != MUGD_OK) return rc;
     if (launches) *launches += pl.p.hot.splits > 1 ? 2 : 1;
     return MUGD_OK;
@@ -240,6 +264,11 @@
 
 extern "C" int mugd_debug_set_tc_tile_n(int bn) {
     mugd::g_tc_force_bn = (bn == 64 || bn == 128) ? bn : 0;
+    return MUGD_OK;
+}
+
+extern "C" int mugd_debug_set_tc_tile_m(int bm) {
+    mugd::g_tc_force_bm = (bm == 128 || bm == 256) ? bm : 0;
     return MUGD_OK;
 }
 
diff --git a/mug_diffusion_b200/csrc/gemm_tc.cuh b/mug_diffusion_b200/csrc/gemm_tc.cuh
--- a/mug_diffusion_b200/csrc/gemm_tc.cuh
+++ b/mug_diffusion_b200/csrc/gemm_tc.cuh
@@ -9,10 +9,8 @@
 
 namespace mugd {
 
-constexpr int TC_BM = 128;
 constexpr int TC_BK = 32;
 constexpr int TC_THREADS = 256;
-constexpr uint32_t TC_A_BYTES = TC_BM * TC_BK * 4;
 
 struct TcParams {
     struct Hot {
@@ -52,17 +50,19 @@
 #else
 #define TC_STAMP(p, k, cta0) do { } while (0)
 #endif
-template <int BN>
+template <int BM, int BN>
 struct TcSmem {
-    static_assert(BN == 64 || BN == 128, "tile widths of the wgmma kernel");
+    static_assert((BM == 128 && (BN == 64 || BN == 128)) || (BM == 256 && BN == 128), "tile shapes of the wgmma kernel");
+    static constexpr uint32_t A_BYTES = BM * TC_BK * 4;
     static constexpr uint32_t B_BYTES = BN * TC_BK * 4;
-    static constexpr uint32_t STAGE_BYTES = TC_A_BYTES + 2 * B_BYTES;
-    static constexpr int STAGES = BN == 128 ? 4 : 6;
+    static constexpr uint32_t STAGE_BYTES = A_BYTES + 2 * B_BYTES;
+    static constexpr int STAGES = BM == 256 ? 3 : BN == 128 ? 4 : 6;
     static constexpr uint32_t TILE_BYTES = STAGES * STAGE_BYTES;
+    static constexpr uint32_t ROWSTAT = TILE_BYTES - BM * 8u;
     static constexpr uint32_t BAR_BYTES = 256;
     static constexpr uint32_t TOTAL = TILE_BYTES + 1024  + BAR_BYTES;
     static_assert(TOTAL <= 227u * 1024u, "shared memory budget");
-    static_assert(128u * (BN + 4) * 4u + 1024u <= TILE_BYTES, "the staged accumulator tile + row statistics must fit the pipeline buffers");
+    static_assert(BM * (BN + 4) * 4u <= ROWSTAT, "the staged accumulator tile + row statistics must fit the pipeline buffers");
 };
 
 template <int SEG>
@@ -124,12 +124,12 @@
     }
 }
 
-template <int BN, int ACT, int GATE, int MODE>
+template <int BM, int BN, int ACT, int GATE, int MODE>
 __device__ __forceinline__ void tc_store_tile(const mugd_gemm& g, uint32_t stage, int m_base, int n0, int rows_valid, const float* rowvec,
                                               uint32_t rowstat, float4 bia, float4 cs) {
     constexpr int SP = BN + 4;
     constexpr int C4 = BN / 4;
-    constexpr int NU = TC_BM * C4 / TC_THREADS;
+    constexpr int NU = BM * C4 / TC_THREADS;
     constexpr int U = NU < 16 ? NU : 16;
     constexpr int SEG = C4 < 32 ? C4 : 32;
     static_assert(TC_THREADS % C4 == 0, "a thread keeps its column quad for the whole tile");
@@ -178,7 +178,7 @@
             }
         }
     };
-    if (n_rows >= TC_BM && n0 + BN <= g.N) pass(std::true_type{});
+    if (n_rows >= BM && n0 + BN <= g.N) pass(std::true_type{});
     else pass(std::false_type{});
 }
 
@@ -203,12 +203,13 @@
     return TC_E_NONE;
 }
 
+template <int BM>
 __device__ __forceinline__ void tc_tile_rows(const TcParams& p, int by, int& b_base, int& l_base, int& rows_valid) {
     const TcParams::Hot& h = p.hot;
-    if (h.Lrows >= TC_BM) {
+    if (h.Lrows >= BM) {
         b_base = by / h.tiles_per_sample;
-        l_base = (by % h.tiles_per_sample) * TC_BM;
-        rows_valid = min(TC_BM, h.Lrows - l_base);
+        l_base = (by % h.tiles_per_sample) * BM;
+        rows_valid = min(BM, h.Lrows - l_base);
     } else {
         b_base = by * h.box_b;
         l_base = 0;
@@ -216,9 +217,9 @@
     }
 }
 
-template <int BN>
+template <int BM, int BN>
 struct TcBars {
-    using S = TcSmem<BN>;
+    using S = TcSmem<BM, BN>;
     static constexpr int COUNT = 2 * S::STAGES;
     static_assert(8 * COUNT <= (int)S::BAR_BYTES, "barrier block");
     uint32_t bars;
@@ -250,24 +251,40 @@
     }
 }
 
-template <int BN, int EPI>
+template <int BN, bool SINGLE>
+__device__ __forceinline__ void tc_kstep_mmas(float (&d)[BN / 2], const TcAFrag& f, uint64_t dbh, uint64_t dbl) {
+#pragma unroll
+    for (int kk = 0; kk < TC_BK / 8; ++kk) {
+        const uint64_t ko = (uint64_t)(kk * 2);
+        if constexpr (SINGLE) {
+            Wgmma<BN>::mma(d, f.hi[kk], dbh + ko);
+        } else {
+            Wgmma<BN>::mma(d, f.lo[kk], dbh + ko);
+            Wgmma<BN>::mma(d, f.hi[kk], dbl + ko);
+            Wgmma<BN>::mma(d, f.hi[kk], dbh + ko);
+        }
+    }
+}
+
+template <int BM, int BN, int EPI>
 __device__ __forceinline__ void gemm_tc_tile(const CUtensorMap* tmA, const CUtensorMap* tmA1, const CUtensorMap* tmA2, const CUtensorMap* tmB,
                                              const CUtensorMap* tmWhi, const CUtensorMap* tmWlo, const TcParams& p, int bx, int by, int bz,
                                              uint32_t base) {
-    using S = TcSmem<BN>;
+    using S = TcSmem<BM, BN>;
     constexpr int STAGES = S::STAGES;
     constexpr int NACC = BN / 2;
-    const TcBars<BN> B(base);
+    const TcBars<BM, BN> B(base);
     auto a_raw = [&](int s) { return base + s * S::STAGE_BYTES; };
-    auto b_hi = [&](int s) { return base + s * S::STAGE_BYTES + TC_A_BYTES; };
+    auto b_hi = [&](int s) { return base + s * S::STAGE_BYTES + S::A_BYTES; };
     auto b_lo = [&](int s) { return b_hi(s) + S::B_BYTES; };
 
     const mugd_gemm& g = p.g;
     const TcParams::Hot& h = p.hot;
     const int warp = threadIdx.x >> 5, lane = threadIdx.x & 31;
+    [[maybe_unused]] const bool cta0 = bx == 0 && by == 0 && bz == 0;
     const int n0 = bx * BN;
     int b_base, l_base, rows_valid;
-    tc_tile_rows(p, by, b_base, l_base, rows_valid);
+    tc_tile_rows<BM>(p, by, b_base, l_base, rows_valid);
     const int m_base = b_base * h.Lrows + l_base;
     const int it_begin = bz * h.it_base + min(bz, h.it_rem);
     const int nit = h.it_base + (bz < h.it_rem ? 1 : 0);
@@ -295,23 +312,24 @@
             tma_load_3d(a_raw(s), tmB, B.full(s), (it - h.it_main) * TC_BK, l_base, b_base);
         }
     };
+    auto prologue = [&]() {
+        const int pro = nit < STAGES ? nit : STAGES;
+        for (int i = 0; i < pro; ++i) issue_w(i);
+        pdl_wait();
+        for (int i = 0; i < pro; ++i) issue_a(i);
+        if (p.pf_bytes > 0) {
+            const int64_t ncta = (int64_t)h.gx * p.gy * h.splits;
+            const int64_t per = (p.pf_bytes / ncta + 15) & ~(int64_t)15;
+            const int64_t off = (((int64_t)bz * p.gy + by) * h.gx + bx) * per;
+            const int64_t n = min(per, p.pf_bytes - off);
+            if (n > 0) {
+                prefetch_l2(reinterpret_cast<const char*>(p.pf_hi) + off, (uint32_t)n);
+                if (p.pf_lo) prefetch_l2(reinterpret_cast<const char*>(p.pf_lo) + off, (uint32_t)n);
+            }
+        }
+    };
     if (warp == 0) {
-        if (elect_one()) {
-            const int pro = nit < STAGES ? nit : STAGES;
-            for (int i = 0; i < pro; ++i) issue_w(i);
-            pdl_wait();
-            for (int i = 0; i < pro; ++i) issue_a(i);
-            if (p.pf_bytes > 0) {
-                const int64_t ncta = (int64_t)h.gx * p.gy * h.splits;
-                const int64_t per = (p.pf_bytes / ncta + 15) & ~(int64_t)15;
-                const int64_t off = (((int64_t)bz * p.gy + by) * h.gx + bx) * per;
-                const int64_t n = min(per, p.pf_bytes - off);
-                if (n > 0) {
-                    prefetch_l2(reinterpret_cast<const char*>(p.pf_hi) + off, (uint32_t)n);
-                    if (p.pf_lo) prefetch_l2(reinterpret_cast<const char*>(p.pf_lo) + off, (uint32_t)n);
-                }
-            }
-        }
+        if (elect_one()) prologue();
         __syncwarp();
     }
 
@@ -330,7 +348,7 @@
         }
         if constexpr (TcEpiTraits<EPI>::MODE == TC_EPI_LN) {
             const int rr = (int)threadIdx.x;
-            if (rr < TC_BM && rr < rows_valid && m_base + rr < g.M) {
+            if (rr < BM && rr < rows_valid && m_base + rr < g.M) {
                 const double2 mo = *reinterpret_cast<const double2*>(g.ln_stats + (int64_t)m_base * 2 + rr * 2);
                 ln_s = mo.x; ln_ss = mo.y;
             }
@@ -338,32 +356,24 @@
     }
 
     const int wg = warp >> 2, g8 = lane >> 2, t4 = lane & 3;
-    const int r0 = wg * 64 + (warp & 3) * 16 + g8;
-    float acc[NACC];
-#pragma unroll
-    for (int j = 0; j < NACC; ++j) acc[j] = 0.f;
+    const int r0 = wg * (BM / 2) + (warp & 3) * 16 + g8;
+    float acc[BM / 128][NACC];
+#pragma unroll
+    for (int b = 0; b < BM / 128; ++b)
+#pragma unroll
+        for (int j = 0; j < NACC; ++j) acc[b][j] = 0.f;
     TcAFrag f0, f1;
+    if constexpr (BM == 256) {
     if (nit > 0) {
         mbar_wait(B.full(0), 0u);
         tc_load_split(a_raw(0), r0, t4, f0);
     }
     auto main_loop = [&](auto single_tag) {
-        constexpr bool SINGLE = decltype(single_tag)::value;
-        auto kstep = [&](int i, const TcAFrag& cur, TcAFrag& nxt) {
+        for (int i = 0; i < nit; ++i) {
             const int s = i % STAGES;
             const uint64_t dbh = wgmma_desc(b_hi(s)), dbl = wgmma_desc(b_lo(s));
             wgmma_fence();
-#pragma unroll
-            for (int kk = 0; kk < TC_BK / 8; ++kk) {
-                const uint64_t ko = (uint64_t)(kk * 2);
-                if constexpr (SINGLE) {
-                    Wgmma<BN>::mma(acc, cur.hi[kk], dbh + ko);
-                } else {
-                    Wgmma<BN>::mma(acc, cur.lo[kk], dbh + ko);
-                    Wgmma<BN>::mma(acc, cur.hi[kk], dbl + ko);
-                    Wgmma<BN>::mma(acc, cur.hi[kk], dbh + ko);
-                }
-            }
+            tc_kstep_mmas<BN, decltype(single_tag)::value>(acc[0], f0, dbh, dbl);
             wgmma_commit();
             wgmma_wait<1>();
             if (i > 0) {
@@ -376,6 +386,42 @@
                     __syncwarp();
                 }
             }
+            tc_load_split(a_raw(s), r0 + 64, t4, f1);
+            wgmma_fence();
+            tc_kstep_mmas<BN, decltype(single_tag)::value>(acc[BM / 128 - 1], f1, dbh, dbl);
+            wgmma_commit();
+            wgmma_wait<1>();
+            if (i + 1 < nit) {
+                mbar_wait(B.full((i + 1) % STAGES), (uint32_t)((i + 1) / STAGES) & 1u);
+                tc_load_split(a_raw((i + 1) % STAGES), r0, t4, f0);
+            }
+        }
+    };
+    if (h.single_pass) main_loop(std::true_type{});
+    else main_loop(std::false_type{});
+    } else {
+    if (nit > 0) {
+        mbar_wait(B.full(0), 0u);
+        tc_load_split(a_raw(0), r0, t4, f0);
+    }
+    auto main_loop = [&](auto single_tag) {
+        auto kstep = [&](int i, const TcAFrag& cur, TcAFrag& nxt) {
+            const int s = i % STAGES;
+            const uint64_t dbh = wgmma_desc(b_hi(s)), dbl = wgmma_desc(b_lo(s));
+            wgmma_fence();
+            tc_kstep_mmas<BN, decltype(single_tag)::value>(acc[0], cur, dbh, dbl);
+            wgmma_commit();
+            wgmma_wait<1>();
+            if (i > 0) {
+                const int j = i - 1, sj = j % STAGES;
+                __syncwarp();
+                if (lane == 0) mbar_arrive(B.empty(sj));
+                if (warp == 0 && j + STAGES < nit) {
+                    mbar_wait(B.empty(sj), (uint32_t)(j / STAGES) & 1u);
+                    if (elect_one()) { issue_w(j + STAGES); issue_a(j + STAGES); }
+                    __syncwarp();
+                }
+            }
             if (i + 1 < nit) {
                 mbar_wait(B.full((i + 1) % STAGES), (uint32_t)((i + 1) / STAGES) & 1u);
                 tc_load_split(a_raw((i + 1) % STAGES), r0, t4, nxt);
@@ -388,32 +434,37 @@
     };
     if (h.single_pass) main_loop(std::true_type{});
     else main_loop(std::false_type{});
+    }
     wgmma_wait<0>();
-    TC_STAMP(p, 2, bx == 0 && by == 0 && bz == 0);
+    TC_STAMP(p, 2, cta0);
     float2 lnrow = make_float2(0.f, 1.f);
     if constexpr (TcEpiTraits<EPI>::MODE == TC_EPI_LN) lnrow = tc_ln_from_moments(ln_s, ln_ss, p.ln_invK, g.ln_eps);
     __syncthreads();
     constexpr int SP = BN + 4;
 #pragma unroll
-    for (int j = 0; j < BN / 8; ++j) {
-        const int c = j * 8 + 2 * t4;
-        sts_f2(base + (uint32_t)(r0 * SP + c) * 4u, acc[4 * j], acc[4 * j + 1]);
-        sts_f2(base + (uint32_t)((r0 + 8) * SP + c) * 4u, acc[4 * j + 2], acc[4 * j + 3]);
+    for (int b = 0; b < BM / 128; ++b) {
+        const int rb = r0 + 64 * b;
+#pragma unroll
+        for (int j = 0; j < BN / 8; ++j) {
+            const int c = j * 8 + 2 * t4;
+            sts_f2(base + (uint32_t)(rb * SP + c) * 4u, acc[b][4 * j], acc[b][4 * j + 1]);
+            sts_f2(base + (uint32_t)((rb + 8) * SP + c) * 4u, acc[b][4 * j + 2], acc[b][4 * j + 3]);
+        }
     }
     if constexpr (TcEpiTraits<EPI>::MODE == TC_EPI_LN) {
-        if (threadIdx.x < TC_BM) sts_f2(base + S::TILE_BYTES - 1024u + (uint32_t)threadIdx.x * 8u, lnrow.x, lnrow.y);
+        if (threadIdx.x < BM) sts_f2(base + S::ROWSTAT + (uint32_t)threadIdx.x * 8u, lnrow.x, lnrow.y);
     }
     __syncthreads();
-    TC_STAMP(p, 3, bx == 0 && by == 0 && bz == 0);
+    TC_STAMP(p, 3, cta0);
     {
         const float* rowvec = g.rowvec ? g.rowvec + (int64_t)epi_step * g.rowvec_step_stride : nullptr;
         if (h.splits > 1) {
             const int tile_lin = by * h.gx + bx;
-            float* wsp = p.ws + ((int64_t)tile_lin * h.splits + bz) * (TC_BM * BN);
+            float* wsp = p.ws + ((int64_t)tile_lin * h.splits + bz) * (BM * BN);
             constexpr int C4 = BN / 4;
             constexpr int U = 8;
 #pragma unroll 1
-            for (int i0 = 0; i0 < TC_BM * C4; i0 += TC_THREADS * U) {
+            for (int i0 = 0; i0 < BM * C4; i0 += TC_THREADS * U) {
                 float4 a4[U];
 #pragma unroll
                 for (int u = 0; u < U; ++u) {
@@ -426,19 +477,19 @@
             }
         } else {
             using E = TcEpiTraits<EPI>;
-            tc_store_tile<BN, E::ACT, E::GATE, E::MODE>(g, base, m_base, n0, rows_valid, rowvec, base + S::TILE_BYTES - 1024u, epi_bias, epi_cs);
-        }
-    }
-    TC_STAMP(p, 4, bx == 0 && by == 0 && bz == 0);
+            tc_store_tile<BM, BN, E::ACT, E::GATE, E::MODE>(g, base, m_base, n0, rows_valid, rowvec, base + S::ROWSTAT, epi_bias, epi_cs);
+        }
+    }
+    TC_STAMP(p, 4, cta0);
 }
 
 template <int BN> constexpr int TC_RED_ROWS = TC_THREADS / (BN / 4);
 
-template <int BN, int EPI>
+template <int BM, int BN, int EPI>
 __device__ __forceinline__ void tc_reduce(const TcParams& p, int blk) {
     constexpr int ACT = TcEpiTraits<EPI>::ACT, GATE = TcEpiTraits<EPI>::GATE, MODE = TcEpiTraits<EPI>::MODE;
     constexpr int C4 = BN / 4;
-    constexpr int BPT = TC_BM / TC_RED_ROWS<BN>;
+    constexpr int BPT = BM / TC_RED_ROWS<BN>;
     constexpr int SEG = C4 < 32 ? C4 : 32;
     constexpr int ZU = 8;
     const mugd_gemm& g = p.g;
@@ -446,7 +497,7 @@
     const int tile_lin = blk / BPT;
     const int bx = tile_lin % h.gx, by = tile_lin / h.gx;
     int b_base, l_base, rows_valid;
-    tc_tile_rows(p, by, b_base, l_base, rows_valid);
+    tc_tile_rows<BM>(p, by, b_base, l_base, rows_valid);
     const int m_base = b_base * h.Lrows + l_base;
     const int c4 = (int)threadIdx.x % C4;
     const int r = (blk % BPT) * TC_RED_ROWS<BN> + (int)threadIdx.x / C4;
@@ -466,14 +517,14 @@
     if constexpr (MODE == TC_EPI_LN) {
         if (ok) mo = *reinterpret_cast<const double2*>(g.ln_stats + (int64_t)m * 2);
     }
-    const float* src = p.ws + ((long long)tile_lin * h.splits) * (TC_BM * BN) + (long long)r * BN + c4 * 4;
+    const float* src = p.ws + ((long long)tile_lin * h.splits) * (BM * BN) + (long long)r * BN + c4 * 4;
     float4 acc = make_float4(0.f, 0.f, 0.f, 0.f);
     for (int z0 = 0; z0 < h.splits; z0 += ZU) {
         float4 t4[ZU];
 #pragma unroll
         for (int u = 0; u < ZU; ++u) {
             t4[u] = make_float4(0.f, 0.f, 0.f, 0.f);
-            if (ok && z0 + u < h.splits) t4[u] = __ldcg(reinterpret_cast<const float4*>(src + (long long)(z0 + u) * (TC_BM * BN)));
+            if (ok && z0 + u < h.splits) t4[u] = __ldcg(reinterpret_cast<const float4*>(src + (long long)(z0 + u) * (BM * BN)));
         }
         if (z0 == 0 && g.rowvec && ok)
             rvv = ld_f4(g.rowvec + (int64_t)step * g.rowvec_step_stride + (int64_t)(m / g.Lout) * g.rowvec_b_stride + n);
@@ -494,13 +545,13 @@
 
 struct TcGeometry {
     TcParams::Hot hot;
-    int BN, gy;
+    int BM, BN, gy;
     int64_t ws_floats;
 };
 struct alignas(64) TcPlanned {
     CUtensorMap maps[6];
     TcParams p;
-    int BN;
+    int BM, BN;
 };
 TcGeometry tc_geometry(const mugd_gemm& g, int sm_count, int forced_split);
 int tc_plan(const DeviceInfo& dev, const mugd_gemm& g, const mugd_gemm* next, TcPlanned* out);
diff --git a/mug_diffusion_b200/lib.py b/mug_diffusion_b200/lib.py
--- a/mug_diffusion_b200/lib.py
+++ b/mug_diffusion_b200/lib.py
@@ -250,6 +250,7 @@
     lib.mugd_set_attention_impl.argtypes = [C.c_void_p, C.c_int]
     lib.mugd_set_s4conv_impl.argtypes = [C.c_void_p, C.c_int]
     lib.mugd_debug_set_tc_tile_n.argtypes = [C.c_int]
+    lib.mugd_debug_set_tc_tile_m.argtypes = [C.c_int]
     lib.mugd_debug_set_tc_cost.argtypes = [C.c_float, C.c_float, C.c_float, C.c_float]
     if os.environ.get("MUGD_TC_COST"):
         lib.mugd_debug_set_tc_cost(*([float(v) for v in os.environ["MUGD_TC_COST"].split(",")] + [0.0] * 4)[:4])
@@ -257,6 +258,8 @@
         lib.mugd_debug_set_tc_tile_n(int(os.environ["MUGD_TC_TILE"]))
     if os.environ.get("MUGD_TC_BN"):
         lib.mugd_debug_set_tc_tile_n(int(os.environ["MUGD_TC_BN"]))
+    if os.environ.get("MUGD_TC_TILE_M"):
+        lib.mugd_debug_set_tc_tile_m(int(os.environ["MUGD_TC_TILE_M"]))
     if os.environ.get("MUGD_PDL") in ("0", "1"):
         lib.mugd_set_pdl(int(os.environ["MUGD_PDL"]))
     _lib = lib
@@ -276,7 +279,7 @@
     "mugd_abi_version", "mugd_last_error", "mugd_create", "mugd_destroy", "mugd_device_info", "mugd_set_gemm_impl",
     "mugd_op_run", "mugd_plan_create", "mugd_plan_run", "mugd_plan_capture", "mugd_plan_replay",
     "mugd_plan_launch_count", "mugd_plan_destroy", "mugd_s4_kernel_gen", "mugd_fill_i32", "mugd_abi_sizes", "mugd_gemm_tc_query",
-    "mugd_set_pdl", "mugd_set_tc_single_pass_tf32", "mugd_set_attention_impl", "mugd_set_s4conv_impl", "mugd_debug_set_tc_tile_n", "mugd_debug_set_tc_cost", "mugd_gemm_tc_variant",
+    "mugd_set_pdl", "mugd_set_tc_single_pass_tf32", "mugd_set_attention_impl", "mugd_set_s4conv_impl", "mugd_debug_set_tc_tile_n", "mugd_debug_set_tc_tile_m", "mugd_debug_set_tc_cost", "mugd_gemm_tc_variant",
     "mugd_debug_set_attention_dump", "mugd_debug_set_tc_timing", "mugd_sample", "mugd_plan_save", "mugd_plan_load", "mugd_plan_regions", "mugd_plan_ops",
     "mugd_melspec", "mugd_grid_scan", "mugd_chart_snap", "mugd_remove_mini_jacks",
     "mugd_sample_staged", "mugd_sample_plms", "mugd_plms_combine",
```

Result: no change. 246.5 (median of 6 runs) (+0.7%).
